# hannes-holey/GaPFlow

Measured on AMD Instinct MI355X. Metric: Mcell-updates/s (fp64), 4096^2 grid, higher is better.
Workload: dtype f64; 1 GPU; 2D journal bearing 4096x4096, fixed DH EOS, all-periodic, adaptive CFL 0.5 (BASELINE.json configs[2]); slabs=1

## Files before the change

gapflow_amd/csrc/api.hip:

```cpp
#include <hip/hip_runtime.h>
#include <algorithm>
#include <cmath>
#include <cstdio>
#include <cstdlib>
#include <cstring>
#include <map>
#include <mutex>
#include <string>
#include <tuple>
#include <vector>

#include "../../include/gapflow_hip.h"
#include "phys_setup.hpp"
#include "step_kernel.hip"
#include "aux_kernels.hip"
#include "step2_kernel.hip"
#include "gp_kernels.hip"
#include "elastic_kernels.hip"
#include "small_kernel.hip"
#include "profile_kernels.hip"

using namespace gpf;

static thread_local std::string g_err;
static const bool g_debug = std::getenv("GPF_DEBUG") != nullptr;
#define DBG(...) do { if (g_debug) { std::fprintf(stderr, "[gpf] " __VA_ARGS__); std::fprintf(stderr, "\n"); std::fflush(stderr); } } while (0)

static int fail(int code, const std::string& msg) {
    g_err = msg;
    return code;
}

struct gpf_handle;
static int enter(gpf_handle* h, bool reads_only = false);

#define HIP_TRY(expr)                                                                                   \
    do {                                                                                                \
        hipError_t e_ = (expr);                                                                         \
        if (e_ != hipSuccess)                                                                           \
            return fail(GPF_ERR_HIP, std::string(#expr) + ": " + hipGetErrorString(e_));               \
    } while (0)

#define GPF_TRY(expr)                                                                                   \
    do {                                                                                                \
        int r_ = (expr);                                                                                \
        if (r_ != GPF_OK) return r_;                                                                    \
    } while (0)

static_assert(sizeof(LogEntry) == sizeof(gpf_scalars_t), "LogEntry must mirror gpf_scalars_t");
static constexpr size_t PLANE_PAD_BYTES = 256;

struct gpf_handle {
    gpf_config cfg;
    Layout L;
    Edges E;
    Phys P;
    hipStream_t stream = nullptr;
    size_t field_bytes = 0;
    double* q[2] = {nullptr, nullptr};
    double* topo = nullptr;
    double* topo_line = nullptr;
    int topo_mode = 0;
    bool topo_hy0 = false;
    double* Ls = nullptr;
    double* g1 = nullptr;
    double* seam = nullptr;
    bool has_seam[2] = {false, false};
    struct { bool on = false; int nranks = 0, rank = 0, rank_lo = -1, rank_hi = -1; char* mine = nullptr;
             char* box[P2P_MAX_RANKS] = {}; unsigned long long* seq = nullptr; } p2p;
    double* halo = nullptr;
    double* beyond = nullptr;
    StepState* st = nullptr;
    Partial* partials = nullptr;
    unsigned int* arrive = nullptr;
    long long p2p_timeout_ticks = P2P_TIMEOUT_TICKS;
    bool split_edges = false;
    bool g1_ready = false;
    Partial* block_partials = nullptr;
    int nghost_blocks = 0;
    ScalarPartial* spart = nullptr;
    int nspart = 0;
    LogEntry* log = nullptr;
    long long log_cap = 0;
    double* stage = nullptr;
    size_t stage_doubles = 0;
    double* fields = nullptr;
    double* work = nullptr;
    struct GpHost {
        bool set = false;
        GpModelDev dev;
        double *Z = nullptr, *alpha = nullptr, *L = nullptr, *Linv = nullptr, *W = nullptr;
        int cap = 0;
        bool has_linv = false;
        double xscale0 = 1.0;
        double inv_scale[GP_MAX_D] = {};
        double yscale_fit = 1.0;
    } gp[3];
    double* gp_state_mean = nullptr;
    bool gp_state_mean_valid = false;
    long long gp_state_mean_step = -1;
    bool gp_state_mean_fresh = false;
    bool open_first_closures = false;
    bool gp_reuse_state_mean = true;
    long long gp_passes[3] = {0, 0, 0}, gp_reused = 0;
    double* gpvar = nullptr;
    double* gpscratch = nullptr;
    int gpscratch_n = 0;
    struct { bool on = false; int px = 0, py = 0, relative = 0; double alpha = 1.0, scale = 1.0; void* plan_f = nullptr; void* plan_b = nullptr;
             double2* greens = nullptr; double2* spec = nullptr; double* dense = nullptr;
             double* u_prev = nullptr; double* h0 = nullptr; double* deformation = nullptr; } el;
    struct { bool on = false; int px = 0, py = 0, nky = 0, nranks = 1, relative = 0;
             int row0 = 0, nrows = 0, k0 = 0, nk = 0, nret = 0, nrows_all = 0, nmain = 0, main_g0 = 0, seam_side = -1, seam_g0 = 0, ref_row = -1;
             double alpha = 1.0, scale = 1.0;
             void* plan_y = nullptr; void* plan_x = nullptr; void* plan_yb = nullptr; int nxg = 0, g_lo = 0;
             double* dense = nullptr; double2* spec = nullptr; double2* send1 = nullptr; double2* recv1 = nullptr; double2* xspec = nullptr;
             double2* greens = nullptr; double2* send2 = nullptr; double2* recv2 = nullptr; double2* line = nullptr; double* ureal = nullptr;
             double* u_prev = nullptr; double* h0 = nullptr; double* deformation = nullptr; double* ref = nullptr; int* rows_all = nullptr; } els;
    double* gptile = nullptr;
    size_t gptile_doubles = 0;
    void* blas = nullptr;
    bool step_open = false;
    int open_parity = 0;
    bool has_q = false, has_topo = false, pre_run_done = false;
    bool prev_state_valid = false;
    long long host_step = 0;
    long long next_step = 0;
    Strip2Geom geom2[2];
    int nchunks2 = 0, nblocks2 = 0, npartials2_cap = 0, nblock_partials_cap = 0;
    bool plan2_valid = false;
    int nt_policy2 = 0;
    int keep_rows2 = 0;
    StepState* st_trial = nullptr;
    double* plan_master = nullptr;
    char plan2_note[400] = "";
};

static int enter(gpf_handle* h, bool reads_only) {
    HIP_TRY(hipSetDevice(h->cfg.device));
    if (!reads_only) h->gp_state_mean_valid = false;
    return GPF_OK;
}

static void make_phys(const gpf_config& c, Phys& P) {
    setup_phys(P, c.U, c.V, c.eta, c.zeta, c.dx, c.dy, c.eos, c.eos_par, c.piezo, c.piezo_par, c.thinning, c.thinning_par);
}

static int blocks_for(long long n, int bs = 256, int cap = 4096) {
    long long b = (n + bs - 1) / bs;
    return (int)std::max<long long>(1, std::min<long long>(b, cap));
}

#ifdef GPF_ONLY_EOS_DH
#define EOS_DISPATCH(eos, ...)                                                                          \
    do {                                                                                                \
        if ((eos) == GPF_EOS_DH) { constexpr int EOS_ = EOS_DH; __VA_ARGS__; }       \
    } while (0)
#else
#define EOS_DISPATCH(eos, ...)                                                                          \
    switch (eos) {                                                                                      \
    case GPF_EOS_DH: { constexpr int EOS_ = EOS_DH; __VA_ARGS__; } break;                              \
    case GPF_EOS_PL: { constexpr int EOS_ = EOS_PL; __VA_ARGS__; } break;                              \
    case GPF_EOS_VDW: { constexpr int EOS_ = EOS_VDW; __VA_ARGS__; } break;                            \
    case GPF_EOS_MT: { constexpr int EOS_ = EOS_MT; __VA_ARGS__; } break;                              \
    case GPF_EOS_CUBIC: { constexpr int EOS_ = EOS_CUBIC; __VA_ARGS__; } break;                        \
    case GPF_EOS_BWR: { constexpr int EOS_ = EOS_BWR; __VA_ARGS__; } break;                            \
    default: { constexpr int EOS_ = EOS_BAYADA; __VA_ARGS__; } break;                                  \
    }
#endif

#define LS_PIEZO_DISPATCH(ls, pz, ...)                                                                  \
    do {                                                                                                \
        if (ls) {                                                                                       \
            constexpr bool LS_ = true;                                                                  \
            if (pz) { constexpr bool PZ_ = true; __VA_ARGS__; } else { constexpr bool PZ_ = false; __VA_ARGS__; }     \
        } else {                                                                                        \
            constexpr bool LS_ = false;                                                                 \
            if (pz) { constexpr bool PZ_ = true; __VA_ARGS__; } else { constexpr bool PZ_ = false; __VA_ARGS__; }     \
        }                                                                                               \
    } while (0)

extern "C" const char* gpf_last_error(void) { return g_err.c_str(); }

extern "C" int gpf_device_count(void) {
    int n = 0;
    if (hipGetDeviceCount(&n) != hipSuccess) return 0;
    return n;
}

static int ensure_stage(gpf_handle* h, size_t doubles) {
    if (h->stage_doubles >= doubles) return GPF_OK;
    if (h->stage) HIP_TRY(hipFree(h->stage));
    h->stage = nullptr; h->stage_doubles = 0;
    HIP_TRY(hipMalloc(&h->stage, doubles * sizeof(double)));
    h->stage_doubles = doubles;
    return GPF_OK;
}

#include "api_fields.inc"

extern "C" int gpf_create(const gpf_config* cfg, gpf_handle** out) {
    if (!cfg || !out) return fail(GPF_ERR_INVALID, "gpf_create: null argument");
    if (cfg->Nx < 1 || cfg->Ny < 1) return fail(GPF_ERR_INVALID, "gpf_create: Nx, Ny must be >= 1");
    if (!(cfg->dx > 0) || !(cfg->dy > 0)) return fail(GPF_ERR_INVALID, "gpf_create: dx, dy must be > 0");
    if (((long long)cfg->Nx + 2) * ((long long)cfg->Ny + 2 + 64) > 2000000000ll)
        return fail(GPF_ERR_INVALID, "gpf_create: more than 2e9 cells per plane; cut the domain into x-slabs (gapflow_amd/slab.py)");
    if (cfg->eos < GPF_EOS_DH || cfg->eos > GPF_EOS_BAYADA) return fail(GPF_ERR_INVALID, "gpf_create: unknown EOS id");
    if (cfg->thinning < 0 || cfg->thinning > GPF_THINNING_CARREAU) return fail(GPF_ERR_INVALID, "gpf_create: unknown shear-thinning id");
    for (int e = 0; e < 4; ++e) {
        int np = 0;
        for (int c = 0; c < 3; ++c) {
            int r = cfg->bc_rule[e][c];
            if (r < 0 || r > 2) return fail(GPF_ERR_INVALID, "gpf_create: bad ghost rule");
            np += (r == GPF_BC_PERIODIC);
        }
        if (np != 0 && np != 3)
            return fail(GPF_ERR_INVALID, "gpf_create: an edge must be periodic for all components or for none "
                                         "(problem.py:682-707 applies the periodic copy only when all three are 'P')");
    }
#ifdef GPF_ONLY_EOS_DH
    if (cfg->eos != GPF_EOS_DH) return fail(GPF_ERR_INVALID, "gpf_create: this build (-DGPF_ONLY_EOS_DH) holds the Dowson-Higginson kernels only");
#endif
    int ndev = 0;
    if (hipGetDeviceCount(&ndev) != hipSuccess || ndev == 0)
        return fail(GPF_ERR_NO_DEVICE, "gpf_create: no HIP device visible (this library has no CPU path)");
    if (cfg->device < 0 || cfg->device >= ndev) return fail(GPF_ERR_INVALID, "gpf_create: device ordinal out of range");
    HIP_TRY(hipSetDevice(cfg->device));

    gpf_handle* h = new gpf_handle();
    h->cfg = *cfg;
    Layout& L = h->L;
    L.Nx = cfg->Nx; L.Ny = cfg->Ny; L.off = 15;
    L.pitch = ((cfg->Ny + 2 + L.off + 15) / 16) * 16;
    if (const char* s = std::getenv("GPF_PITCH_PAD")) L.pitch += (std::atoi(s) / 16) * 16;
    L.plane = (long long)(cfg->Nx + 2) * L.pitch;
    if (const char* s = std::getenv("GPF_PLANE_PAD")) L.plane += (std::atoll(s) & ~1ll);
    for (int e = 0; e < 4; ++e) {
        for (int c = 0; c < 3; ++c) h->E.rule[e][c] = cfg->bc_rule[e][c];
        h->E.value[e] = cfg->bc_value[e];
    }
    h->E.halo[0] = cfg->halo_lo; h->E.halo[1] = cfg->halo_hi;
    h->split_edges = std::getenv("GPF_STEP_UNFUSED_EDGES") != nullptr;
    h->gp_reuse_state_mean = std::getenv("GPF_GP_NO_STATE_MEAN") == nullptr;
    make_phys(*cfg, h->P);

    const size_t plane_b = (size_t)L.plane * sizeof(double);
    auto cleanup = [&](int code) { gpf_destroy(h); return code; };
#define HIP_TRY_C(expr)                                                                                 \
    do {                                                                                                \
        hipError_t e_ = (expr);                                                                         \
        if (e_ != hipSuccess)                                                                           \
            return cleanup(fail(GPF_ERR_HIP, std::string(#expr) + ": " + hipGetErrorString(e_)));      \
    } while (0)
    h->field_bytes = (3 * plane_b + PLANE_PAD_BYTES + 255) & ~(size_t)255;
    for (int b = 0; b < 2; ++b) {
        HIP_TRY_C(field_malloc((void**)&h->q[b], h->field_bytes));
        if (field_zero(0, h->q[b], h->field_bytes) != GPF_OK) { gpf_destroy(h); return GPF_ERR_HIP; }
    }
    HIP_TRY_C(field_malloc((void**)&h->topo, h->field_bytes));
    if (field_zero(0, h->topo, h->field_bytes) != GPF_OK) { gpf_destroy(h); return GPF_ERR_HIP; }
    HIP_TRY_C(hipDeviceSynchronize());
    const size_t g1n = (size_t)3 * L.pitch + (size_t)3 * (L.Nx + 2);
    HIP_TRY_C(hipMalloc(&h->g1, g1n * sizeof(double)));
    HIP_TRY_C(hipMemset(h->g1, 0, g1n * sizeof(double)));
    HIP_TRY_C(hipMalloc(&h->st, sizeof(StepState)));
    HIP_TRY_C(hipMemset(h->st, 0, sizeof(StepState)));
    h->nghost_blocks = std::max(1, std::min(64, (2 * (L.Ny + 2) + 2 * L.Nx + 255) / 256));
    HIP_TRY_C(hipMalloc(&h->arrive, 4 * sizeof(unsigned int)));
    HIP_TRY_C(hipMemset(h->arrive, 0, 4 * sizeof(unsigned int)));
    HIP_TRY_C(hipMalloc(&h->block_partials, 1024 * sizeof(Partial)));
    h->nspart = 1024;
    HIP_TRY_C(hipMalloc(&h->spart, (size_t)(h->nspart + 8) * sizeof(ScalarPartial)));
    HIP_TRY_C(hipMemset(h->spart, 0, (size_t)(h->nspart + 8) * sizeof(ScalarPartial)));
    h->log_cap = 4096;
    HIP_TRY_C(hipMalloc(&h->log, (size_t)h->log_cap * sizeof(LogEntry)));
#undef HIP_TRY_C
    *out = h;
    return GPF_OK;
}

extern "C" int gpf_destroy(gpf_handle* h) {
    if (!h) return GPF_OK;
    hipSetDevice(h->cfg.device);
    hipStreamSynchronize(h->stream);
    for (void* p : {(void*)h->q[0], (void*)h->q[1], (void*)h->topo, (void*)h->plan_master}) field_free(p);
    void* ptrs[] = {h->topo_line, h->Ls, h->g1, h->seam, h->halo, h->beyond, h->st, h->partials, h->arrive, h->block_partials, h->spart,
                    h->log, h->stage, h->fields, h->work, h->st_trial, h->gpvar, h->gp_state_mean, h->gpscratch, h->gptile,
                    h->gp[0].Z, h->gp[0].alpha, h->gp[0].L, h->gp[1].Z, h->gp[1].alpha, h->gp[1].L,
                    h->gp[2].Z, h->gp[2].alpha, h->gp[2].L, h->gp[0].Linv, h->gp[1].Linv, h->gp[2].Linv, h->gp[0].W, h->gp[1].W, h->gp[2].W};
    if (h->blas && roclibs().ok) roclibs().destroy(h->blas);
    if (h->el.plan_f) fftlib().destroy(h->el.plan_f);
    if (h->el.plan_b) fftlib().destroy(h->el.plan_b);
    for (void* p : {(void*)h->el.greens, (void*)h->el.spec, (void*)h->el.dense, (void*)h->el.u_prev})
        if (p) hipFree(p);
    for (void* pl : {h->els.plan_y, h->els.plan_x, h->els.plan_yb})
        if (pl) fftlib().destroy(pl);
    for (void* p : {(void*)h->els.dense, (void*)h->els.spec, (void*)h->els.send1, (void*)h->els.recv1, (void*)h->els.xspec, (void*)h->els.greens,
                    (void*)h->els.send2, (void*)h->els.recv2, (void*)h->els.line, (void*)h->els.ureal, (void*)h->els.u_prev, (void*)h->els.ref,
                    (void*)h->els.rows_all})
        if (p) hipFree(p);
    for (int r = 0; r < h->p2p.nranks; ++r)
        if (h->p2p.box[r] && r != h->p2p.rank) hipIpcCloseMemHandle(h->p2p.box[r]);
    if (h->p2p.mine) hipFree(h->p2p.mine);
    if (h->p2p.seq) hipFree(h->p2p.seq);
    for (void* p : ptrs)
        if (p) hipFree(p);
    delete h;
    return GPF_OK;
}

extern "C" int gpf_set_stream(gpf_handle* h, void* s) {
    if (!h) return fail(GPF_ERR_INVALID, "null handle");
    h->stream = (hipStream_t)s;
    return GPF_OK;
}

static int field_ncomp(int field) {
    switch (field) {
    case GPF_FIELD_Q: return 3;
    case GPF_FIELD_TOPO: return 3;
    case GPF_FIELD_EXTRA: return 1;
    case GPF_FIELD_PRESSURE: return 1;
    case GPF_FIELD_TAU_AVG: return 3;
    case GPF_FIELD_WALL_LOWER: return 6;
    case GPF_FIELD_WALL_UPPER: return 6;
    case GPF_FIELD_PRESSURE_VAR: case GPF_FIELD_WALL_XZ_VAR: case GPF_FIELD_WALL_YZ_VAR: return 1;
    case GPF_FIELD_DEFORMATION: return 1;
    }
    return 0;
}

static int current_parity(gpf_handle* h, int* par) {
    StepState s;
    HIP_TRY(hipMemcpyAsync(&s, h->st, sizeof(s), hipMemcpyDeviceToHost, h->stream));
    HIP_TRY(hipStreamSynchronize(h->stream));
    *par = s.parity;
    return GPF_OK;
}

static int ensure_fields(gpf_handle* h) {
    if (h->fields) return GPF_OK;
    HIP_TRY(hipMalloc(&h->fields, (size_t)16 * h->L.plane * sizeof(double)));
    HIP_TRY(hipMemsetAsync(h->fields, 0, (size_t)16 * h->L.plane * sizeof(double), h->stream));
    return GPF_OK;
}

extern "C" int gpf_upload(gpf_handle* h, int field, const double* host, size_t count) {
    if (!h || !host) return fail(GPF_ERR_INVALID, "gpf_upload: null argument");
    GPF_TRY(enter(h));
    const Layout& L = h->L;
    const int nc = field_ncomp(field);
    if (field != GPF_FIELD_Q && field != GPF_FIELD_TOPO && field != GPF_FIELD_EXTRA)
        return fail(GPF_ERR_INVALID, "gpf_upload: only q, topography and the extra field are inputs");
    const size_t ncell = (size_t)(L.Nx + 2) * (L.Ny + 2);
    if (count != ncell * nc) return fail(GPF_ERR_INVALID, "gpf_upload: count does not match ncomp*(Nx+2)*(Ny+2)");
    double* dst = nullptr;
    if (field == GPF_FIELD_Q) {
        int par = 0;
        GPF_TRY(current_parity(h, &par));
        dst = h->q[par];
    } else if (field == GPF_FIELD_TOPO) {
        dst = h->topo;
    } else {
        bool nz = false;
        for (size_t i = 0; i < count && !nz; ++i) nz = host[i] != 0.0;
        if (!nz && !h->Ls) return GPF_OK;
        if (!h->Ls) { HIP_TRY(hipMalloc(&h->Ls, (size_t)L.plane * sizeof(double) + PLANE_PAD_BYTES)); h->plan2_valid = false; }
        HIP_TRY(hipMemsetAsync(h->Ls, 0, (size_t)L.plane * sizeof(double), h->stream));
        dst = h->Ls;
    }
    if (field == GPF_FIELD_TOPO) {
        const int nx = L.Nx + 2, ny = L.Ny + 2;
        bool xonly = true, yonly = true;
        for (int c = 0; c < 3 && (xonly || yonly); ++c)
            for (int ix = 0; ix < nx && (xonly || yonly); ++ix) {
                const double* row = host + ((size_t)c * nx + ix) * ny;
                const double* row0 = host + (size_t)c * nx * ny;
                for (int iy = 0; iy < ny; ++iy) {
                    if (std::memcmp(&row[iy], &row[0], 8) != 0) xonly = false;
                    if (std::memcmp(&row[iy], &row0[iy], 8) != 0) yonly = false;
                }
            }
        const int mode = xonly ? 1 : (yonly ? 2 : 0);
        if (mode != h->topo_mode) { h->plan2_valid = false; }
        h->topo_mode = (h->el.on || h->els.on) ? 0 : mode;
        if (mode) {
            const int n = mode == 1 ? nx : ny;
            std::vector<double> line((size_t)3 * n);
            for (int c = 0; c < 3; ++c)
                for (int i = 0; i < n; ++i)
                    line[(size_t)c * n + i] = mode == 1 ? host[((size_t)c * nx + i) * ny] : host[(size_t)c * nx * ny + i];
            bool hy0 = mode == 1;
            for (int i = 0; i < n && hy0; ++i) hy0 = line[(size_t)2 * n + i] == 0.0;
            if (hy0 != h->topo_hy0) h->plan2_valid = false;
            h->topo_hy0 = hy0;
            if (!h->topo_line) HIP_TRY(hipMalloc(&h->topo_line, (size_t)3 * (std::max(nx, ny)) * sizeof(double)));
            HIP_TRY(hipMemcpy(h->topo_line, line.data(), line.size() * sizeof(double), hipMemcpyHostToDevice));
        }
    }
    GPF_TRY(ensure_stage(h, count));
    HIP_TRY(hipMemcpyAsync(h->stage, host, count * sizeof(double), hipMemcpyHostToDevice, h->stream));
    hipLaunchKernelGGL(k_pack, dim3(blocks_for((long long)count)), dim3(256), 0, h->stream, h->stage, dst, L, nc);
    HIP_TRY(hipGetLastError());
    HIP_TRY(hipStreamSynchronize(h->stream));
    if (field == GPF_FIELD_Q) h->has_q = true;
    h->g1_ready = false;
    h->prev_state_valid = false;
    if (field == GPF_FIELD_TOPO) h->has_topo = true;
    return GPF_OK;
}

extern "C" int gpf_download(gpf_handle* h, int field, double* host, size_t count) {
    if (!h || !host) return fail(GPF_ERR_INVALID, "gpf_download: null argument");
    GPF_TRY(enter(h, true));
    const Layout& L = h->L;
    const int nc = field_ncomp(field);
    if (nc == 0) return fail(GPF_ERR_INVALID, "gpf_download: unknown field id");
    const size_t ncell = (size_t)(L.Nx + 2) * (L.Ny + 2);
    if (count != ncell * nc) return fail(GPF_ERR_INVALID, "gpf_download: count does not match ncomp*(Nx+2)*(Ny+2)");
    const double* src = nullptr;
    switch (field) {
    case GPF_FIELD_Q: {
        int par = 0;
        GPF_TRY(current_parity(h, &par));
        src = h->q[par];
        break;
    }
    case GPF_FIELD_TOPO: src = h->topo; break;
    case GPF_FIELD_EXTRA:
        if (!h->Ls) { std::memset(host, 0, count * sizeof(double)); return GPF_OK; }
        src = h->Ls; break;
    case GPF_FIELD_DEFORMATION:
        if (!h->el.on && !h->els.on) { std::memset(host, 0, count * sizeof(double)); return GPF_OK; }
        src = h->el.on ? h->el.deformation : h->els.deformation; break;
    case GPF_FIELD_PRESSURE_VAR: case GPF_FIELD_WALL_XZ_VAR: case GPF_FIELD_WALL_YZ_VAR:
        if (!h->gpvar) return fail(GPF_ERR_STATE, "gpf_download: no GP variance has been computed");
        src = h->gpvar + (size_t)(field - GPF_FIELD_PRESSURE_VAR) * L.plane;
        break;
    default:
        if (!h->fields) return fail(GPF_ERR_STATE, "gpf_download: derived fields requested before gpf_update_closures");
        src = h->fields + (field == GPF_FIELD_PRESSURE ? 0 : field == GPF_FIELD_TAU_AVG ? 1 : field == GPF_FIELD_WALL_LOWER ? 4 : 10) * L.plane;
    }
    GPF_TRY(ensure_stage(h, count));
    hipLaunchKernelGGL(k_unpack, dim3(blocks_for((long long)count)), dim3(256), 0, h->stream, src, h->stage, L, nc);
    HIP_TRY(hipGetLastError());
    HIP_TRY(hipMemcpyAsync(host, h->stage, count * sizeof(double), hipMemcpyDeviceToHost, h->stream));
    HIP_TRY(hipStreamSynchronize(h->stream));
    return GPF_OK;
}

static FieldPtrs field_ptrs(gpf_handle* h) {
    FieldPtrs F;
    F.p = h->fields; F.tau = h->fields + h->L.plane; F.lower = h->fields + 4 * h->L.plane; F.upper = h->fields + 10 * h->L.plane;
    return F;
}

static int gp_launch_mean(gpf_handle* h, int which, const double* q, bool with_grad, double* c2_out);
static int read_state(gpf_handle* h, StepState& s);

static const double* beyond_rows(gpf_handle* h, const double* q) {
    if (!h->beyond || (h->E.halo[0] != 1 && h->E.halo[1] != 1)) return nullptr;
    const bool working = h->step_open && q == h->q[h->open_parity ^ 1];
    return h->beyond + (working ? 2 * h->L.pitch : 0);
}

static int launch_fields(gpf_handle* h, const double* q, bool pressure_mean_cached = false) {
    GPF_TRY(ensure_fields(h));
    const Layout& L = h->L;
    const long long n = (long long)(L.Nx + 2) * (L.Ny + 2);
    FieldPtrs F = field_ptrs(h);
    EOS_DISPATCH(h->cfg.eos, {
        if (h->cfg.thinning != GPF_THINNING_NONE) {
            hipLaunchKernelGGL((k_pressure<EOS_>), dim3(blocks_for(n)), dim3(256), 0, h->stream, q, F.p, L, h->P);
            if ((h->E.halo[0] == 1 || h->E.halo[1] == 1) && !h->beyond)
                return fail(GPF_ERR_STATE, "shear thinning on a slab: upload the rows beyond the halo first (gpf_upload_beyond)");
            const double* by = beyond_rows(h, q);
            if (h->Ls) hipLaunchKernelGGL((k_fields_thinning<EOS_, true>), dim3(blocks_for(n)), dim3(256), 0, h->stream, q, h->topo, h->Ls, F, L, h->P, h->cfg.dx, h->cfg.dy, h->E.halo[0], h->E.halo[1], by);
            else hipLaunchKernelGGL((k_fields_thinning<EOS_, false>), dim3(blocks_for(n)), dim3(256), 0, h->stream, q, h->topo, (const double*)nullptr, F, L, h->P, h->cfg.dx, h->cfg.dy, h->E.halo[0], h->E.halo[1], by);
        } else if (h->Ls) hipLaunchKernelGGL((k_fields<EOS_, true>), dim3(blocks_for(n)), dim3(256), 0, h->stream, q, h->topo, h->Ls, F, L, h->P);
        else hipLaunchKernelGGL((k_fields<EOS_, false>), dim3(blocks_for(n)), dim3(256), 0, h->stream, q, h->topo, (const double*)nullptr, F, L, h->P);
    });
    HIP_TRY(hipGetLastError());
    for (int w = 0; w < 3; ++w) {
        if (!h->gp[w].set) continue;
        if (w == 0 && pressure_mean_cached) {
            HIP_TRY(hipMemcpyAsync(F.p, h->gp_state_mean, (size_t)L.plane * sizeof(double), hipMemcpyDeviceToDevice, h->stream));
            h->gp_reused += 1;
        } else GPF_TRY(gp_launch_mean(h, w, q, false, nullptr));
    }
    return GPF_OK;
}

extern "C" int gpf_update_closures(gpf_handle* h) {
    if (!h) return fail(GPF_ERR_INVALID, "null handle");
    if (!h->has_q || !h->has_topo) return fail(GPF_ERR_STATE, "gpf_update_closures: upload q and topography first");
    GPF_TRY(enter(h));
    int par = 0;
    GPF_TRY(current_parity(h, &par));
    if (h->prev_state_valid && !h->E.halo[0] && !h->E.halo[1]) {
        const Layout& L = h->L;
        StepState s;
        GPF_TRY(read_state(h, s));
        double* w = h->q[par ^ 1];
        const long long n = (long long)(L.Nx + 2) * (L.Ny + 2);
        const int nb = blocks_for(n);
        if (!h->work) HIP_TRY(hipMalloc(&h->work, (size_t)9 * L.plane * sizeof(double)));
        GPF_TRY(launch_fields(h, w));
        double *fx = h->work, *fy = h->work + 3 * L.plane, *src = h->work + 6 * L.plane;
        FieldPtrs F = field_ptrs(h);
        const int mc = h->cfg.mc_order;
        const int sw = mc == 0 ? (((s.step - 1) % 2 == 0) ? 1 : -1) : mc;
        const int dir = ((sw + 1) / 2) ? 1 : -1;
        hipLaunchKernelGGL(k_fluxdiff, dim3(nb), dim3(256), 0, h->stream, w, F.p, F.tau, dir, fx, fy, L);
        hipLaunchKernelGGL(k_source, dim3(nb), dim3(256), 0, h->stream, w, h->topo, F.tau, F.lower, F.upper, src, L);
        hipLaunchKernelGGL(k_axpy, dim3(nb), dim3(256), 0, h->stream, w, fx, fy, src, (const double*)&h->st->dt_last, h->cfg.dx, h->cfg.dy, L);
        hipLaunchKernelGGL(k_bc_x, dim3((L.Ny + 2 + 255) / 256), dim3(256), 0, h->stream, w, L, h->E);
        hipLaunchKernelGGL(k_bc_y, dim3((L.Nx + 2 + 255) / 256), dim3(256), 0, h->stream, w, L, h->E);
        HIP_TRY(hipGetLastError());
        GPF_TRY(launch_fields(h, w));
        h->prev_state_valid = false;
    } else {
        GPF_TRY(launch_fields(h, h->q[par]));
    }
    HIP_TRY(hipStreamSynchronize(h->stream));
    return GPF_OK;
}

static int launch_scalars(gpf_handle* h, const double* q, ScalarPartial* total, bool need_sound_speed = true) {
    const Layout& L = h->L;
    const int row0 = h->E.halo[0] == 1 ? 1 : 0, row1 = h->E.halo[1] == 1 ? L.Nx : L.Nx + 1;
    const long long n = (long long)(row1 - row0 + 1) * (L.Ny + 2);
    const int nb = blocks_for(n, 256, h->nspart);
    EOS_DISPATCH(h->cfg.eos, {
        hipLaunchKernelGGL((k_scalars<EOS_>), dim3(nb), dim3(256), 0, h->stream, q, h->topo, L, h->P, row0, row1, h->spart);
    });
    HIP_TRY(hipGetLastError());
    hipLaunchKernelGGL(k_scalars_final, dim3(1), dim3(256), 0, h->stream, h->spart, nb, total);
    HIP_TRY(hipGetLastError());
    if (h->gp[0].set && need_sound_speed) GPF_TRY(gp_launch_mean(h, 0, q, true, &total->c2));
    return GPF_OK;
}

static void fill_scalars(const StepState& s, const ScalarPartial* sp, double dxdy, gpf_scalars_t* out) {
    out->step = s.step; out->simtime = s.simtime; out->dt = s.dt;
    out->ekin = sp ? sp->ekin : s.ekin; out->ekin_old = s.ekin_old; out->residual = s.residual;
    out->v_max = std::sqrt(sp ? sp->v2 : s.vmax2);
    out->v_sound = (sp && ((int)sp->flags & 4)) ? std::nan("") : std::sqrt(sp ? sp->c2 : s.c2max);
    out->mass = sp ? sp->mass * dxdy : 0.0;
    out->invalid = s.invalid; out->converged = s.converged;
}

extern "C" int gpf_scalars(gpf_handle* h, gpf_scalars_t* out) {
    if (!h || !out) return fail(GPF_ERR_INVALID, "gpf_scalars: null argument");
    if (!h->has_q || !h->has_topo) return fail(GPF_ERR_STATE, "gpf_scalars: upload q and topography first");
    GPF_TRY(enter(h, true));
    int par = 0;
    GPF_TRY(current_parity(h, &par));
    ScalarPartial* tot = h->spart + h->nspart;
    h->gp_state_mean_fresh = false;
    GPF_TRY(launch_scalars(h, h->q[par], tot));
    ScalarPartial sp; StepState s;
    HIP_TRY(hipMemcpyAsync(&sp, tot, sizeof(sp), hipMemcpyDeviceToHost, h->stream));
    HIP_TRY(hipMemcpyAsync(&s, h->st, sizeof(s), hipMemcpyDeviceToHost, h->stream));
    HIP_TRY(hipStreamSynchronize(h->stream));
    if (h->gp_state_mean_fresh && s.parity == par) {
        h->gp_state_mean_valid = true;
        h->gp_state_mean_step = s.step;
    }
    h->gp_state_mean_fresh = false;
    fill_scalars(s, &sp, h->cfg.dx * h->cfg.dy, out);
    return GPF_OK;
}

static int write_state(gpf_handle* h, const StepState& s) {
    HIP_TRY(hipMemcpyAsync(h->st, &s, sizeof(s), hipMemcpyHostToDevice, h->stream));
    HIP_TRY(hipStreamSynchronize(h->stream));
    return GPF_OK;
}
static int read_state(gpf_handle* h, StepState& s) {
    HIP_TRY(hipMemcpyAsync(&s, h->st, sizeof(s), hipMemcpyDeviceToHost, h->stream));
    HIP_TRY(hipStreamSynchronize(h->stream));
    return GPF_OK;
}

extern "C" int gpf_set_ekin_old(gpf_handle* h, double v) {
    if (!h) return fail(GPF_ERR_INVALID, "null handle");
    StepState s;
    GPF_TRY(read_state(h, s));
    s.ekin_old = v;
    return write_state(h, s);
}

extern "C" int gpf_set_dt(gpf_handle* h, double dt) {
    if (!h) return fail(GPF_ERR_INVALID, "null handle");
    StepState s;
    GPF_TRY(read_state(h, s));
    s.dt = dt;
    h->g1_ready = false;
    return write_state(h, s);
}

extern "C" int gpf_pre_run(gpf_handle* h) {
    if (!h) return fail(GPF_ERR_INVALID, "null handle");
    if (!h->has_q || !h->has_topo) return fail(GPF_ERR_STATE, "gpf_pre_run: upload q and topography first");
    GPF_TRY(enter(h));
    gpf_scalars_t sc;
    GPF_TRY(gpf_scalars(h, &sc));
    StepState s;
    GPF_TRY(read_state(h, s));
    const gpf_config& c = h->cfg;
    s.hmin = std::min(c.dx, c.dy);
    s.tol = c.tol; s.CFL = c.CFL; s.adaptive = c.adaptive; s.mc_order = c.mc_order; s.max_it = c.max_it;
    s.step = 0; s.simtime = 0.0; s.residual = 1.0;
    s.rbuf[0] = 1.0; s.rcount = 1; s.rhead = 0;
    s.converged = (1.0 < c.tol) ? 1 : 0;
    s.invalid = 0;
    s.dt_last = 0.0;
    if (!h->pre_run_done) s.ekin_old = sc.ekin;
    s.ekin = sc.ekin;
    s.vmax2 = sc.v_max * sc.v_max; s.c2max = sc.v_sound * sc.v_sound;
    const double dt_crit = s.hmin / (sc.v_max + sc.v_sound);
    s.dt = c.adaptive ? c.CFL * dt_crit : c.dt_fixed;
    GPF_TRY(write_state(h, s));
    h->pre_run_done = true;
    h->g1_ready = false;
    h->prev_state_valid = false;
    h->host_step = 0; h->next_step = 0;
    return GPF_OK;
}

static int topo_mode_of(const gpf_handle* h) {
    if (h->Ls != nullptr || h->cfg.piezo != 0 || std::getenv("GPF_TOPO_PLANES")) return 0;
    if (h->topo_mode == 1 && h->topo_hy0 && !std::getenv("GPF_TOPO_GENERIC")) return 3;
    return h->topo_mode;
}

typedef void (*step2_kernel_t)(const Step2Args, const Phys);

static step2_kernel_t step2_kernel(int eos, bool has_ls, bool piezo, int D, int topo_mode) {
    step2_kernel_t k = nullptr;
    EOS_DISPATCH(eos, {
        if (piezo) {
            if (has_ls) k = D > 0 ? k_step2<EOS_, true, true, 1, 0> : k_step2<EOS_, true, true, -1, 0>;
            else k = D > 0 ? k_step2<EOS_, false, true, 1, 0> : k_step2<EOS_, false, true, -1, 0>;
        } else if (has_ls) {
            k = D > 0 ? k_step2<EOS_, true, false, 1, 0> : k_step2<EOS_, true, false, -1, 0>;
        } else if (topo_mode == 1) {
            k = D > 0 ? k_step2<EOS_, false, false, 1, 1> : k_step2<EOS_, false, false, -1, 1>;
        } else if (topo_mode == 2) {
            k = D > 0 ? k_step2<EOS_, false, false, 1, 2> : k_step2<EOS_, false, false, -1, 2>;
        } else if (topo_mode == 3) {
            k = D > 0 ? k_step2<EOS_, false, false, 1, 3> : k_step2<EOS_, false, false, -1, 3>;
        } else {
            k = D > 0 ? k_step2<EOS_, false, false, 1, 0> : k_step2<EOS_, false, false, -1, 0>;
        }
    });
    return k;
}

static Strip2Geom strip2_geom(const Layout& L, int D) {
    Strip2Geom G;
    const int e = (D < 0 && (L.Ny & 1)) ? 1 : 0;
    for (int k = 0; k < 2; ++k) {
        G.w0 = -1 - e - 4 * k;
        G.s_ghost = (L.Ny - G.w0 - 1) / STRIP2;
        const int p_ny = L.Ny - G.w0 - STRIP2 * G.s_ghost;
        G.lane_ghost = (p_ny + 1) >> 1; G.slot_ghost = (p_ny + 1) & 1;
        if (G.lane_ghost + 2 <= 63) break;
    }
    G.nstrips = G.s_ghost + 1;
    G.lane_wrap = G.lane_ghost + 1;
    const int p0 = -G.w0;
    G.wrap_ma = (p0 % 2 == 0) ? 0 : -1;
    const int d = 1 - G.wrap_ma;
    G.wrap_src_lane = G.lane_wrap + d / 2; G.wrap_src_slot = d & 1;
    return G;
}

static bool step2_fused(const gpf_handle* h) { return !h->split_edges; }

#include "api_plan.inc"

#ifndef GPF_SLAB_COMMIT_BLOCKS
#define GPF_SLAB_COMMIT_BLOCKS 24
#endif
constexpr int SLAB_COMMIT_BLOCKS = GPF_SLAB_COMMIT_BLOCKS;

static P2PArgs p2p_args(gpf_handle* h, bool on) {
    P2PArgs c;
    c.on = on ? 1 : 0; c.nranks = h->p2p.nranks; c.rank = h->p2p.rank; c.rank_lo = h->p2p.rank_lo; c.rank_hi = h->p2p.rank_hi;
    for (int r = 0; r < P2P_MAX_RANKS; ++r) c.box[r] = h->p2p.box[r];
    c.seq = h->p2p.seq; c.qa = h->q[0]; c.qb = h->q[1];
    return c;
}

static int ghost_args(gpf_handle* h, int honor_stop, GhostArgs& g) {
    const Layout& L = h->L;
    g.qa = h->q[0]; g.qb = h->q[1]; g.topo = h->topo; g.Ls = h->Ls;
    for (int e = 0; e < 2; ++e) {
        g.seam[e] = nullptr;
        if (h->E.halo[e] == 2) {
            if (!h->has_seam[e]) return fail(GPF_ERR_STATE, "periodic slab seam: call gpf_set_seam_topo for this edge first");
            g.seam[e] = h->seam + (size_t)e * 8 * L.pitch;
        }
    }
    g.g1x = h->g1; g.g1y = h->g1 + 3 * L.pitch;
    g.st = h->st; g.L = L; g.E = h->E; g.honor_stop = honor_stop;
    return GPF_OK;
}

static void fill_step2_args(gpf_handle* h, Step2Args& a2, int D, int honor_stop, long long log_base, double* slab_out, bool p2p) {
    const Layout& L = h->L;
    const bool fused = step2_fused(h);
    const Strip2Geom& G2 = h->geom2[D > 0 ? 0 : 1];
    a2.qa = h->q[0]; a2.qb = h->q[1]; a2.topo = h->topo; a2.topo_line = h->topo_line; a2.Ls = h->Ls;
    a2.g1x = h->g1; a2.g1y = h->g1 + 3 * L.pitch;
    a2.st = h->st; a2.partials = h->partials; a2.block_partials = h->block_partials; a2.arrive = h->arrive;
    a2.log = h->log; a2.log_base = log_base; a2.log_cap = h->log_cap;
    a2.L = L; a2.E = h->E; a2.G = G2; a2.nchunks = h->nchunks2; a2.fused = (fused ? 1 : 0) | (h->nt_policy2 >= 1 ? 2 : 0) | (h->nt_policy2 >= 2 ? 4 : 0) |
               (h->nt_policy2 >= 1 ? h->keep_rows2 << 3 : 0); a2.honor_stop = honor_stop;
    const bool slab = slab_out != nullptr;
    for (int e = 0; e < 2; ++e) a2.seam[e] = (h->E.halo[e] == 2 && h->has_seam[e]) ? h->seam + (size_t)e * 8 * L.pitch : nullptr;
    a2.out = slab_out; a2.msg = (slab && !p2p) ? h->halo : nullptr; a2.p2p = p2p_args(h, p2p);
}

static int enqueue_step(gpf_handle* h, int honor_stop, long long log_base, double* slab_out,
                        hipEvent_t ev0 = nullptr, hipEvent_t ev1 = nullptr, bool p2p = false) {
    const Layout& L = h->L;
    const int mc = h->cfg.mc_order;
    const int D = mc == 0 ? ((h->next_step % 2 == 0) ? 1 : -1) : (((mc + 1) / 2) ? 1 : -1);
    GPF_TRY(plan_step2(h, D));
    h->next_step += 1;
    const bool fused = step2_fused(h);
    const Strip2Geom& G2 = h->geom2[D > 0 ? 0 : 1];
    const int np_step = G2.nstrips * h->nchunks2;
    GhostArgs g;
    GPF_TRY(ghost_args(h, honor_stop, g));
    Step2Args a2;
    fill_step2_args(h, a2, D, honor_stop, log_base, slab_out, p2p);
    const bool slab = slab_out != nullptr;
    FinishArgs f;
    f.partials = h->partials; f.st = h->st;
    f.log = h->log; f.log_base = log_base; f.log_cap = h->log_cap; f.out = slab_out; f.honor_stop = honor_stop;
    f.L = L; f.E = h->E;
    f.p2p = p2p_args(h, p2p);
    f.arrive = h->arrive; f.msg = slab ? h->halo : nullptr;
    f.nstep_partials = np_step; f.block_partials = h->block_partials;
    GhostFillArgs gf;
    gf.qa = h->q[0]; gf.qb = h->q[1]; gf.st = h->st;
    gf.L = L; gf.E = h->E; gf.honor_stop = honor_stop;

    const int ntiles = (L.Nx + L.Ny + 63) / 64;
    const dim3 ggrid(std::min(ntiles, 512));
    const int nsend = slab ? std::min((6 * L.pitch + 1023) / 1024, 256) : 0;
    WaitArgs w;
    w.qa = h->q[0]; w.qb = h->q[1]; w.st = h->st; w.log = h->log; w.log_base = log_base; w.log_cap = h->log_cap;
    w.L = L; w.E = h->E; w.honor_stop = honor_stop; w.arrive = h->arrive + 1; w.timeout_ticks = h->p2p_timeout_ticks; w.p2p = f.p2p;
    w.gathered = nullptr; w.msg_len = 0; w.nranks = 0; w.rank_lo = w.rank_hi = -1; w.stage1 = fused ? 0 : 1;
    const bool has_ls = h->Ls != nullptr;
    if (fused) {
        const step2_kernel_t k2 = step2_kernel(h->cfg.eos, h->Ls != nullptr, h->cfg.piezo != 0, D, topo_mode_of(h));
        if (ev0) hipEventRecord(ev0, h->stream);
        hipLaunchKernelGGL(k2, dim3(h->nblocks2), dim3(256), 0, h->stream, a2, h->P);
        if (ev1) hipEventRecord(ev1, h->stream);
        if (p2p) {
            const dim3 cgrid(SLAB_COMMIT_BLOCKS);
            EOS_DISPATCH(h->cfg.eos, {
                hipLaunchKernelGGL((k_begin_slab<EOS_, false, false, false, true>), cgrid, dim3(256), 0, h->stream, g, w, h->P);
            });
        }
        h->g1_ready = false;
        HIP_TRY(hipGetLastError());
        return GPF_OK;
    }
    EOS_DISPATCH(h->cfg.eos, {
        if (!h->g1_ready) {
            if (topo_mode_of(h) == 3) hipLaunchKernelGGL((k_ghost_stage1<EOS_, false, false, true>), ggrid, dim3(256), 0, h->stream, g, h->P);
            else LS_PIEZO_DISPATCH(has_ls, h->cfg.piezo != 0, hipLaunchKernelGGL((k_ghost_stage1<EOS_, LS_, PZ_, false>), ggrid, dim3(256), 0, h->stream, g, h->P));
        }
        if (ev0) hipEventRecord(ev0, h->stream);
        hipLaunchKernelGGL(step2_kernel(h->cfg.eos, h->Ls != nullptr, h->cfg.piezo != 0, D, topo_mode_of(h)), dim3(h->nblocks2), dim3(256), 0, h->stream, a2, h->P);
        if (ev1) hipEventRecord(ev1, h->stream);
        hipLaunchKernelGGL((k_ghost_fill<EOS_>), dim3(h->nghost_blocks + nsend), dim3(256), 0, h->stream, gf, f, h->nghost_blocks, h->P);
        if (p2p) {
            if (topo_mode_of(h) == 3) hipLaunchKernelGGL((k_begin_slab<EOS_, false, false, true, true>), ggrid, dim3(256), 0, h->stream, g, w, h->P);
            else LS_PIEZO_DISPATCH(has_ls, h->cfg.piezo != 0, hipLaunchKernelGGL((k_begin_slab<EOS_, LS_, PZ_, false, true>), ggrid, dim3(256), 0, h->stream, g, w, h->P));
        }
    });
    h->g1_ready = p2p;
    HIP_TRY(hipGetLastError());
    return GPF_OK;
}

static bool small_grid_eligible(gpf_handle* h) {
    static const bool off = getenv("GPF_SMALL_GRID") && atoi(getenv("GPF_SMALL_GRID")) == 0;
    const long long nc = (long long)(h->L.Nx + 2) * (h->L.Ny + 2);
    return !off && nc * SMALL_DOUBLES_PER_CELL * 8 <= 150 * 1024 && h->cfg.thinning == GPF_THINNING_NONE && !h->E.halo[0] && !h->E.halo[1] &&
           !h->gp[0].set && !h->gp[1].set && !h->gp[2].set && !h->el.on;
}

static int enqueue_small_steps(gpf_handle* h, int nsteps, int honor_stop, long long log_base) {
    const Layout& L = h->L;
    SmallArgs a;
    a.qa = h->q[0]; a.qb = h->q[1]; a.topo = h->topo; a.Ls = h->Ls; a.st = h->st;
    a.log = h->log; a.log_base = log_base; a.log_cap = h->log_cap; a.L = L; a.E = h->E; a.nsteps = nsteps; a.honor_stop = honor_stop;
    const size_t lds = (size_t)(L.Nx + 2) * (L.Ny + 2) * SMALL_DOUBLES_PER_CELL * 8;
    EOS_DISPATCH(h->cfg.eos, {
        if (h->Ls) {
            HIP_TRY(hipFuncSetAttribute((const void*)k_small_steps<EOS_, true>, hipFuncAttributeMaxDynamicSharedMemorySize, (int)lds));
            hipLaunchKernelGGL((k_small_steps<EOS_, true>), dim3(1), dim3(512), lds, h->stream, a, h->P);
        } else {
            HIP_TRY(hipFuncSetAttribute((const void*)k_small_steps<EOS_, false>, hipFuncAttributeMaxDynamicSharedMemorySize, (int)lds));
            hipLaunchKernelGGL((k_small_steps<EOS_, false>), dim3(1), dim3(512), lds, h->stream, a, h->P);
        }
    });
    HIP_TRY(hipGetLastError());
    h->next_step += nsteps;
    h->g1_ready = false;
    return GPF_OK;
}

extern "C" int gpf_step(gpf_handle* h, int64_t n, int honor_stop, gpf_scalars_t* log, int64_t log_capacity,
                        int64_t* n_executed) {
    if (!h) return fail(GPF_ERR_INVALID, "null handle");
    if (!h->pre_run_done) return fail(GPF_ERR_STATE, "gpf_step: call gpf_pre_run first (Problem._pre_run, problem.py:412)");
    if (h->E.halo[0] || h->E.halo[1]) return fail(GPF_ERR_STATE, "gpf_step: this handle is a slab; use gpf_step_local / gpf_step_commit");
    if (h->cfg.thinning != GPF_THINNING_NONE)
        return fail(GPF_ERR_STATE, "gpf_step: shear thinning needs grad p (a wider stencil than the fused step has); use the stage-wise calls");
    if (n < 0) return fail(GPF_ERR_INVALID, "gpf_step: n < 0");
    GPF_TRY(enter(h));
    int64_t done = 0, logged = 0;
    const bool small = small_grid_eligible(h);
    while (done < n) {
        const int64_t batch = std::min<int64_t>(n - done, h->log_cap);
        const long long base = h->host_step;
        if (small) GPF_TRY(enqueue_small_steps(h, (int)batch, honor_stop, base));
        else for (int64_t i = 0; i < batch; ++i) GPF_TRY(enqueue_step(h, honor_stop, base, nullptr));
        StepState s;
        GPF_TRY(read_state(h, s));
        const long long ran = s.step - base;
        const long long entries = ran + ((s.invalid && ran < batch) ? 1 : 0);
        if (log && entries > 0) {
            const long long take = std::min<long long>(entries, log_capacity - logged);
            if (take > 0) {
                HIP_TRY(hipMemcpy(log + logged, h->log, (size_t)take * sizeof(LogEntry), hipMemcpyDeviceToHost));
                logged += take;
            }
        }
        h->host_step = s.step; h->next_step = s.step;
        h->prev_state_valid = ran >= 1 && !s.invalid;
        done += batch;
        if (ran < batch) break;
    }
    if (n_executed) *n_executed = h->host_step;
    return GPF_OK;
}

extern "C" int gpf_step_timed(gpf_handle* h, int64_t n, double* kernel_ms, double* total_ms) {
    if (!h || !kernel_ms || !total_ms) return fail(GPF_ERR_INVALID, "gpf_step_timed: null argument");
    if (!h->pre_run_done) return fail(GPF_ERR_STATE, "gpf_step_timed: call gpf_pre_run first");
    if (n < 1 || n > h->log_cap) return fail(GPF_ERR_INVALID, "gpf_step_timed: 1 <= n <= 4096");
    GPF_TRY(enter(h));
    std::vector<hipEvent_t> ev(2 * n + 2);
    for (auto& e : ev) HIP_TRY(hipEventCreate(&e));
    HIP_TRY(hipEventRecord(ev[2 * n], h->stream));
    int rc = GPF_OK;
    for (int64_t i = 0; i < n && rc == GPF_OK; ++i) rc = enqueue_step(h, 0, h->host_step, nullptr, ev[2 * i], ev[2 * i + 1]);
    HIP_TRY(hipEventRecord(ev[2 * n + 1], h->stream));
    HIP_TRY(hipStreamSynchronize(h->stream));
    double sum = 0.0;
    float ms = 0.f;
    for (int64_t i = 0; i < n; ++i) {
        HIP_TRY(hipEventElapsedTime(&ms, ev[2 * i], ev[2 * i + 1]));
        sum += ms;
    }
    HIP_TRY(hipEventElapsedTime(&ms, ev[2 * n], ev[2 * n + 1]));
    *kernel_ms = sum; *total_ms = ms;
    for (auto& e : ev) hipEventDestroy(e);
    StepState s;
    GPF_TRY(read_state(h, s));
    h->prev_state_valid = s.step > h->host_step && !s.invalid;
    h->host_step = s.step; h->next_step = s.step;
    return rc;
}

#include "api_unfused_step.inc"
#include "api_operators.inc"
#include "api_slab_allgather.inc"
#include "api_elastic.inc"
#include "api_slab_p2p.inc"
#include "api_gp.inc"
#include "api_stagewise.inc"
#include "api_slab_stagewise.inc"
#include "api_slab_elastic.inc"
#include "api_profiles.inc"
```

gapflow_amd/csrc/api_plan.inc:

```

constexpr int K2_LONG_MARCH_ROWS = 100;

static int plan_apply(gpf_handle* h, int nchunks, int nt, int keep = 0) {
    const Layout& L = h->L;
    const int nstrips = std::max(h->geom2[0].nstrips, h->geom2[1].nstrips);
    nchunks = std::max(1, std::min(nchunks, std::max(1, L.Nx / 4)));
    h->nchunks2 = nchunks;
    h->nt_policy2 = nt;
    h->keep_rows2 = nt >= 1 ? std::max(0, std::min(7, keep)) : 0;
    const int nwaves = nstrips * nchunks;
    h->nblocks2 = (((nwaves + 3) / 4) + 7) / 8 * 8;
    if (nwaves > h->npartials2_cap) {
        if (h->partials) HIP_TRY(hipFree(h->partials));
        h->partials = nullptr;
        HIP_TRY(hipMalloc(&h->partials, (size_t)nwaves * sizeof(Partial)));
        HIP_TRY(hipMemset(h->partials, 0, (size_t)nwaves * sizeof(Partial)));
        h->npartials2_cap = nwaves;
    }
    if (h->nblocks2 > h->nblock_partials_cap) {
        const int cap = std::max(1024, h->nblocks2);
        if (h->block_partials) HIP_TRY(hipFree(h->block_partials));
        h->block_partials = nullptr;
        HIP_TRY(hipMalloc(&h->block_partials, (size_t)cap * sizeof(Partial)));
        h->nblock_partials_cap = cap;
    }
    return GPF_OK;
}

static void fill_step2_args(gpf_handle* h, Step2Args& a2, int D, int honor_stop, long long log_base, double* slab_out, bool p2p);

static int plan_trial(gpf_handle* h, int D, float* us, int reps = 6, bool both = false) {
    static const int parity_value[2] = {0, 1};
    if (!h->st_trial) HIP_TRY(hipMalloc(&h->st_trial, sizeof(StepState)));
    h->prev_state_valid = false;
    both = both && h->plan_master != nullptr;
    int par = 0;
    if (both) GPF_TRY(current_parity(h, &par));
    Step2Args a2;
    fill_step2_args(h, a2, D, 0, 0, nullptr, false);
    a2.st = h->st_trial; a2.log = nullptr;
    const step2_kernel_t k2 = step2_kernel(h->cfg.eos, h->Ls != nullptr, h->cfg.piezo != 0, D, topo_mode_of(h));
    hipEvent_t e0, e1;
    HIP_TRY(hipEventCreate(&e0)); HIP_TRY(hipEventCreate(&e1));
    float total = 0.f;
    for (int r = -1; r < reps; ++r) {
        HIP_TRY(hipMemcpyAsync(h->st_trial, h->st, sizeof(StepState), hipMemcpyDeviceToDevice, h->stream));
        if (both && ((r + 1) & 1))
            HIP_TRY(hipMemcpyAsync(&h->st_trial->parity, &parity_value[par ^ 1], sizeof(int), hipMemcpyHostToDevice, h->stream));
        HIP_TRY(hipEventRecord(e0, h->stream));
        hipLaunchKernelGGL(k2, dim3(h->nblocks2), dim3(256), 0, h->stream, a2, h->P);
        HIP_TRY(hipEventRecord(e1, h->stream));
        HIP_TRY(hipEventSynchronize(e1));
        float ms = 0.f;
        HIP_TRY(hipEventElapsedTime(&ms, e0, e1));
        if (r >= 0) total += ms;
    }
    hipEventDestroy(e0); hipEventDestroy(e1);
    if (both) GPF_TRY(field_copy(h->stream, h->q[par], h->plan_master, h->field_bytes));
    HIP_TRY(hipGetLastError());
    *us = total / reps * 1e3f;
    return GPF_OK;
}

static float placement_best_seen(const gpf_handle* h, int D, float mine) {
    static std::mutex lock;
    static std::map<std::tuple<int, int, int, int, int, int, int>, float> seen;
    const auto key = std::make_tuple(h->L.Nx, h->L.Ny, h->cfg.eos, topo_mode_of(h), D, h->Ls ? 1 : 0, h->cfg.piezo != 0 ? 1 : 0);
    std::lock_guard<std::mutex> g(lock);
    float& v = seen[key];
    if (mine > 0.f && (v == 0.f || mine < v)) v = mine;
    return v;
}

static int plan_placement(gpf_handle* h, int D, std::string& note) {
    const char* env_tries = std::getenv("GPF_PLACEMENT_TRIES");
    const int fixed = env_tries ? std::atoi(env_tries) : -1;
    if (fixed == 0 || !h->plan_master) return GPF_OK;
    const bool print = std::getenv("GPF_PLACEMENT_PRINT") && std::atoi(std::getenv("GPF_PLACEMENT_PRINT")) != 0;
    int par = 0;
    GPF_TRY(current_parity(h, &par));
    const bool planes = topo_mode_of(h) == 0;
    double* const master = h->plan_master;
    std::vector<double*> pool = {h->q[par], h->q[par ^ 1]};
    std::vector<char> holds_state = {1, 0};
    std::vector<float> w = {0.f, 0.f};
    auto trial = [&](int i, int j, float* us, bool both) -> int {
        if (!holds_state[i]) {
            GPF_TRY(field_copy(h->stream, pool[i], master, h->field_bytes));
            holds_state[i] = 1;
        }
        holds_state[j] = 0;
        h->q[par] = pool[i]; h->q[par ^ 1] = pool[j];
        return plan_trial(h, D, us, 6, both);
    };
    float best_w = 0.f;
    for (int round = 0; round < (fixed > 0 ? 1 : 5); ++round) {
        int want = fixed > 0 ? fixed : 12;
        size_t free_b = 0, total_b = 0;
        HIP_TRY(hipMemGetInfo(&free_b, &total_b));
        while (want > 0 && (size_t)want * h->field_bytes + (2ull << 30) > free_b) --want;
        const size_t first = pool.size();
        for (int k = 0; k < want; ++k) {
            double* b = nullptr;
            if (field_malloc((void**)&b, h->field_bytes) != hipSuccess) { (void)hipGetLastError(); break; }
            GPF_TRY(field_zero(h->stream, b, h->field_bytes));
            pool.push_back(b); holds_state.push_back(0); w.push_back(0.f);
        }
        if (pool.size() == first) break;
        float batch_best = 0.f;
        for (size_t k = first; k < pool.size(); ++k) {
            GPF_TRY(trial(0, (int)k, &w[k], false));
            if (batch_best == 0.f || w[k] < batch_best) batch_best = w[k];
        }
        const bool paid = best_w == 0.f || batch_best < 0.99f * best_w;
        if (best_w == 0.f || batch_best < best_w) best_w = batch_best;
        const float known = placement_best_seen(h, D, 0.f);
        if (round >= 1 && !paid && !(known > 0.f && best_w > 1.03f * known)) break;
    }
    (void)placement_best_seen(h, D, best_w);
    const int n = (int)pool.size();
    if (n == 2) return GPF_OK;
    GPF_TRY(trial(0, 1, &w[1], false));
    GPF_TRY(trial(1, 0, &w[0], false));
    std::vector<int> order(n);
    for (int k = 0; k < n; ++k) order[k] = k;
    std::stable_sort(order.begin(), order.end(), [&](int x, int y) { return w[x] < w[y]; });
    const int m = std::min(n, 4);
    float own_pair = 0.f;
    GPF_TRY(trial(0, 1, &own_pair, true));
    int bi = 0, bj = 1;
    float best = own_pair, worst = own_pair;
    std::string pairs;
    for (int i = 0; i < m; ++i)
        for (int j = i + 1; j < m; ++j) {
            const int x = std::min(order[i], order[j]), y = std::max(order[i], order[j]);
            if (x == 0 && y == 1) continue;
            float t = 0.f;
            GPF_TRY(trial(x, y, &t, true));
            if (print) { char b2[40]; std::snprintf(b2, sizeof b2, " (%d,%d) %.1f", x, y, t); pairs += b2; }
            if (t < best) { best = t; bi = x; bj = y; }
            worst = std::max(worst, t);
        }
    if (print) {
        std::fprintf(stderr, "[gpf] placement: us per step writing each buffer (0, 1: the handle's own):");
        for (int k = 0; k < n; ++k) std::fprintf(stderr, " %.1f", w[k]);
        std::fprintf(stderr, "\n[gpf] placement: pairs, both directions: (0,1) %.1f%s\n", own_pair, pairs.c_str());
    }
    char buf[200];
    std::snprintf(buf, sizeof buf, " placement: %d buffers, written %.0f .. %.0f us, pair kept %.0f, the handle's own %.0f", n,
                  *std::min_element(w.begin(), w.end()), *std::max_element(w.begin(), w.end()), best, own_pair);
    note = buf;
    std::vector<double*> rest;
    for (int k = 0; k < n; ++k) if (k != bi && k != bj) rest.push_back(pool[k]);
    float us = 0.f;
    if (planes) {
        double* const own = h->topo;
        double* best_home = own;
        float best_t = 0.f;
        std::string seen;
        for (size_t k = 0; k <= std::min<size_t>(rest.size(), 3); ++k) {
            double* cand = k == 0 ? own : rest[k - 1];
            if (cand != own) GPF_TRY(field_copy(h->stream, cand, own, h->field_bytes));
            h->topo = cand;
            float t = 0.f;
            GPF_TRY(trial(bi, bj, &t, true));
            std::snprintf(buf, sizeof buf, " %.0f", t);
            seen += buf;
            if (k == 0 || t < best_t) { best_t = t; best_home = cand; }
        }
        note += "; gap planes:" + seen;
        if (best_home != own) {
            rest.erase(std::find(rest.begin(), rest.end(), best_home));
            rest.push_back(own);
        }
        h->topo = best_home;
    }
    GPF_TRY(trial(bi, bj, &us, true));
    HIP_TRY(hipStreamSynchronize(h->stream));
    for (double* b : rest) field_free(b);
    h->q[par] = pool[bi]; h->q[par ^ 1] = pool[bj];
    return GPF_OK;
}

static const char* const NT_NAME[3] = {"plain loads and stores", "non-temporal stores", "non-temporal loads and stores"};
constexpr int K2_KEEP_ROWS_DEFAULT = 4;
static const int K2_KEEP_CANDIDATES[2] = {3, 4};
static std::string keep_note(const gpf_handle* h) {
    if (h->nt_policy2 < 1) return "";
    char buf[64];
    std::snprintf(buf, sizeof buf, ", keep %d/8 rows on-die", h->keep_rows2);
    return buf;
}
static int plan_step2(gpf_handle* h, int D) {
    if (h->plan2_valid) return GPF_OK;
    const Layout& L = h->L;
    h->geom2[0] = strip2_geom(L, 1);
    h->geom2[1] = strip2_geom(L, -1);
    const int nstrips = std::max(h->geom2[0].nstrips, h->geom2[1].nstrips);
    int per_cu = 0, ncu = 0;
    HIP_TRY(hipOccupancyMaxActiveBlocksPerMultiprocessor(&per_cu, (const void*)step2_kernel(h->cfg.eos, h->Ls != nullptr, h->cfg.piezo != 0, 1, topo_mode_of(h)), 256, 0));
    HIP_TRY(hipDeviceGetAttribute(&ncu, hipDeviceAttributeMultiprocessorCount, h->cfg.device));
    const int all_resident = std::max(1, std::max(1, per_cu * ncu) * 4 / nstrips);
    const int one_per_simd = (ncu * 4) / nstrips;
    const double streamed = (double)L.plane * 8.0 * (6 + (topo_mode_of(h) == 0 ? 3 : 0) + (h->Ls ? 1 : 0));
    const bool nt_possible = streamed > 192.0 * 1024 * 1024;
    const char* env_chunks = std::getenv("GPF_CHUNKS");
    const char* env_nt = std::getenv("GPF_NT") ? std::getenv("GPF_NT") : std::getenv("GPF_NT_STORES");
    const char* env_tune = std::getenv("GPF_PLAN_TUNE");
    int nchunks = all_resident;
    if (one_per_simd >= 1 && L.Nx / one_per_simd >= K2_LONG_MARCH_ROWS) nchunks = one_per_simd;
    int nt = nt_possible ? 2 : 0;
    if (env_chunks && std::atoi(env_chunks) > 0) nchunks = std::atoi(env_chunks);
    if (env_nt) nt = std::max(0, std::min(2, std::atoi(env_nt)));
    const char* env_keep = std::getenv("GPF_KEEP_ROWS");
    int keep = nt_possible ? K2_KEEP_ROWS_DEFAULT : 0;
    if (env_keep) keep = std::max(0, std::min(7, std::atoi(env_keep)));
    const bool tune = !(env_tune && std::atoi(env_tune) == 0) && !h->split_edges && h->pre_run_done && (long long)L.Nx * L.Ny >= (1ll << 20) &&
                      one_per_simd >= 1 && L.Nx / one_per_simd >= 16 && !(env_chunks && env_nt);
    if (!tune) {
        GPF_TRY(plan_apply(h, nchunks, nt, keep));
        std::snprintf(h->plan2_note, sizeof h->plan2_note, "%d chunks per strip, %s%s (rule of thumb%s)", h->nchunks2,
                      NT_NAME[h->nt_policy2], keep_note(h).c_str(), (env_chunks || env_nt || env_keep) ? ", pinned by the environment" : "");
        h->plan2_valid = true;
        return GPF_OK;
    }
    std::string placement_note;
    GPF_TRY(plan_apply(h, nchunks, nt));
    {
        int par = 0;
        GPF_TRY(current_parity(h, &par));
        if (field_malloc((void**)&h->plan_master, h->field_bytes) == hipSuccess)
            GPF_TRY(field_copy(h->stream, h->plan_master, h->q[par], h->field_bytes));
        else { (void)hipGetLastError(); h->plan_master = nullptr; }
    }
    {
        float unused = 0.f;
        const double step_s = 1.1e-11 * (double)L.Nx * L.Ny + 1e-5;
        GPF_TRY(plan_trial(h, D, &unused, (int)std::min(200.0, std::max(8.0, 0.012 / step_s))));
    }
    float best = 0.f;
    int best_chunks = nchunks;
    int best_nt = nt;
    int best_keep = 0;
    std::string seen, keep_seen;
    auto pick_plan = [&]() -> int {
        best = 0.f;
        seen.clear();
        for (int c : {one_per_simd, all_resident}) {
            if (env_chunks && std::atoi(env_chunks) > 0) c = std::atoi(env_chunks);
            for (int pol = 0; pol < (nt_possible && !env_nt ? 3 : 1); ++pol) {
                const int cand_nt = env_nt ? nt : pol;
                GPF_TRY(plan_apply(h, c, cand_nt));
                float us = 0.f;
                GPF_TRY(plan_trial(h, D, &us, 6, true));
                char buf[48];
                std::snprintf(buf, sizeof buf, " %d/%s %.0f", h->nchunks2, cand_nt == 2 ? "nt" : cand_nt == 1 ? "nts" : "plain", us);
                seen += buf;
                if (best == 0.f || us < best) { best = us; best_chunks = c; best_nt = cand_nt; }
            }
            if ((env_chunks && std::atoi(env_chunks) > 0) || one_per_simd == all_resident) break;
        }
        best_keep = 0;
        keep_seen.clear();
        if (best_nt >= 1) {
            if (env_keep) best_keep = keep;
            else if (nt_possible) {
                char buf[48];
                std::snprintf(buf, sizeof buf, " 0 %.0f", best);
                keep_seen = buf;
                float best_k = best;
                for (int k : K2_KEEP_CANDIDATES) {
                    GPF_TRY(plan_apply(h, best_chunks, best_nt, k));
                    float us = 0.f;
                    GPF_TRY(plan_trial(h, D, &us, 6, true));
                    std::snprintf(buf, sizeof buf, ", %d %.0f", k, us);
                    keep_seen += buf;
                    if (us < best_k) { best_k = us; best_keep = k; }
                }
            }
        }
        return plan_apply(h, best_chunks, best_nt, best_keep);
    };
    const bool verify = std::getenv("GPF_PLACEMENT_PRINT") && std::atoi(std::getenv("GPF_PLACEMENT_PRINT")) >= 2;
    auto stamp = [&](const char* when) {
        if (!verify) return;
        int par = 0;
        if (current_parity(h, &par) != GPF_OK) return;
        std::fprintf(stderr, "[gpf] %-28s q[par] %p %016llx   master %p %016llx\n", when, (void*)h->q[par], field_checksum(h->stream, h->q[par], h->field_bytes),
                     (void*)h->plan_master, h->plan_master ? field_checksum(h->stream, h->plan_master, h->field_bytes) : 0ull);
    };
    stamp("before the first plan");
    GPF_TRY(pick_plan());
    stamp("after the first plan");
    const std::string first_seen = seen;
    GPF_TRY(plan_placement(h, D, placement_note));
    stamp("after the placement");
    if (!placement_note.empty()) GPF_TRY(pick_plan());
    stamp("after the second plan");
    HIP_TRY(hipStreamSynchronize(h->stream));
    field_free(h->plan_master);
    h->plan_master = nullptr;
    GPF_TRY(plan_apply(h, best_chunks, best_nt, best_keep));
    const std::string kept = keep_note(h) + (keep_seen.empty() ? (env_keep && h->nt_policy2 >= 1 ? " (pinned by the environment)" : "")
                                                               : " (timed, us: k" + keep_seen + ")");
    std::snprintf(h->plan2_note, sizeof h->plan2_note, "%d chunks per strip, %s%s (timed, us:%s;%s%s%s)", h->nchunks2,
                  NT_NAME[h->nt_policy2], kept.c_str(), seen.c_str(), placement_note.c_str(),
                  placement_note.empty() ? "" : "; before the placement:", placement_note.empty() ? "" : first_seen.c_str());
    DBG("plan_step2: %s", h->plan2_note);
    h->plan2_valid = true;
    return GPF_OK;
}

extern "C" const char* gpf_plan_note(gpf_handle* h) { return h ? h->plan2_note : ""; }
```

gapflow_amd/csrc/aux_kernels.hip:

```cpp
#include <hip/hip_runtime.h>
#include "device_types.hpp"

namespace gpf {

__global__ void k_pack(const double* __restrict__ src, double* __restrict__ dst, Layout L, int ncomp) {
    const long long ncell = (long long)(L.Nx + 2) * (L.Ny + 2);
    for (long long i = blockIdx.x * (long long)blockDim.x + threadIdx.x; i < ncell * ncomp;
         i += (long long)gridDim.x * blockDim.x) {
        const int c = (int)(i / ncell);
        const long long r = i - c * ncell;
        const int ix = (int)(r / (L.Ny + 2)), iy = (int)(r - (long long)ix * (L.Ny + 2));
        dst[c * L.plane + L.at(ix, iy)] = src[i];
    }
}

__global__ void k_unpack(const double* __restrict__ src, double* __restrict__ dst, Layout L, int ncomp) {
    const long long ncell = (long long)(L.Nx + 2) * (L.Ny + 2);
    for (long long i = blockIdx.x * (long long)blockDim.x + threadIdx.x; i < ncell * ncomp;
         i += (long long)gridDim.x * blockDim.x) {
        const int c = (int)(i / ncell);
        const long long r = i - c * ncell;
        const int ix = (int)(r / (L.Ny + 2)), iy = (int)(r - (long long)ix * (L.Ny + 2));
        dst[i] = src[c * L.plane + L.at(ix, iy)];
    }
}

__device__ __forceinline__ double ghost_x(const double* q, const Layout& L, const Edges& E, int e, int c, int iy) {
    const int r = E.rule[e][c];
    const int adj = e == 0 ? 1 : L.Nx;
    const int src = (r == BC_P) ? (e == 0 ? L.Nx : 1) : adj;
    const double v = q[c * L.plane + L.at(src, iy)];
    return r == BC_D ? 2.0 * E.value[e] - v : v;
}
__device__ __forceinline__ double ghost_y(const double* q, const Layout& L, const Edges& E, int e, int c, int ix) {
    const int r = E.rule[e][c];
    const int adj = e == 2 ? 1 : L.Ny;
    const int src = (r == BC_P) ? (e == 2 ? L.Ny : 1) : adj;
    const double v = q[c * L.plane + L.at(ix, src)];
    return r == BC_D ? 2.0 * E.value[e] - v : v;
}

__global__ void k_bc_x(double* q, Layout L, Edges E) {
    const int iy = blockIdx.x * blockDim.x + threadIdx.x;
    if (iy > L.Ny + 1) return;
    for (int e = 0; e < 2; ++e) {
        if (E.halo[e]) continue;
        const int ix = e == 0 ? 0 : L.Nx + 1;
        double v[3];
        for (int c = 0; c < 3; ++c) v[c] = ghost_x(q, L, E, e, c, iy);
        for (int c = 0; c < 3; ++c) q[c * L.plane + L.at(ix, iy)] = v[c];
    }
}
__global__ void k_bc_y(double* q, Layout L, Edges E) {
    const int ix = blockIdx.x * blockDim.x + threadIdx.x;
    if (ix > L.Nx + 1) return;
    for (int e = 2; e < 4; ++e) {
        const int iy = e == 2 ? 0 : L.Ny + 1;
        double v[3];
        for (int c = 0; c < 3; ++c) v[c] = ghost_y(q, L, E, e, c, ix);
        for (int c = 0; c < 3; ++c) q[c * L.plane + L.at(ix, iy)] = v[c];
    }
}

struct Acc {
    double ekin, v2, c2, mass;
    int flags;
    __device__ __forceinline__ void zero() { ekin = 0; v2 = 0; c2 = 0; mass = 0; flags = 0; }
    template <int EOS>
    __device__ __forceinline__ void cell(double r, double jx, double jy, double h, const Phys& P, double w = 1.0) {
        const double v = (jx * jx + jy * jy) / r;
        ekin += w * (v * 0.5);
        v2 = nanmax(v2, v);
        const double c = eos_c2<EOS>(r, P);
        if (!(c >= 0.0)) flags |= 4;
        c2 = fmax(c2, c);
        mass += w * (r * h);
        if (r != r || jx != jx || jy != jy) flags |= 1;
        if (r < 0.0) flags |= 2;
    }
    __device__ __forceinline__ void merge(const Acc& o) {
        ekin += o.ekin; v2 = nanmax(v2, o.v2); c2 = nanmax(c2, o.c2); mass += o.mass; flags |= o.flags;
    }
};

__device__ __forceinline__ Acc wave_reduce(Acc a) {
    for (int s = 32; s >= 1; s >>= 1) {
        Acc o;
        o.ekin = __shfl_down(a.ekin, s); o.v2 = __shfl_down(a.v2, s); o.c2 = __shfl_down(a.c2, s);
        o.mass = __shfl_down(a.mass, s); o.flags = __shfl_down(a.flags, s);
        a.merge(o);
    }
    return a;
}

__device__ __forceinline__ Acc block_reduce(Acc a, Acc* smem) {
    a = wave_reduce(a);
    const int lane = threadIdx.x & 63, w = threadIdx.x >> 6;
    if (lane == 0) smem[w] = a;
    __syncthreads();
    Acc r; r.zero();
    if (threadIdx.x == 0) {
        for (int i = 0; i < (int)(blockDim.x >> 6); ++i) r.merge(smem[i]);
    }
    __syncthreads();
    return r;
}

struct ScalarPartial { double ekin, v2, c2, mass, flags; };

template <int EOS>
__global__ __launch_bounds__(256) void k_scalars(const double* q, const double* topo, Layout L, Phys P, int row0,
                                                 int row1, ScalarPartial* out) {
    __shared__ Acc sm[4];
    Acc a; a.zero();
    const long long w = L.Ny + 2;
    const long long n = (long long)(row1 - row0 + 1) * w;
    for (long long i = blockIdx.x * (long long)blockDim.x + threadIdx.x; i < n; i += (long long)gridDim.x * blockDim.x) {
        const int ix = row0 + (int)(i / w), iy = (int)(i % w);
        const long long o = L.at(ix, iy);
        a.cell<EOS>(q[o], q[o + L.plane], q[o + 2 * L.plane], topo[o], P);
    }
    a = block_reduce(a, sm);
    if (threadIdx.x == 0) {
        ScalarPartial p = {a.ekin, a.v2, a.c2, a.mass, (double)a.flags};
        out[blockIdx.x] = p;
    }
}

__device__ __forceinline__ double critical_dt(const StepState* st, double v2, double c2) {
    return st->hmin / (sqrt(v2) + sqrt(c2));
}

__device__ inline void commit_step(StepState* st, double ekin, double v2, double c2, int flags, LogEntry* log,
                                   long long log_base, long long log_cap) {
    if (flags & 4) c2 = __builtin_nan("");
    flags &= 3;
    if (flags) {
        st->invalid = (flags & 1) ? 1 : 2;
    } else {
        const double dt_crit = critical_dt(st, v2, c2);
        const double cfl = st->dt / dt_crit;
        const double res = fabs(ekin - st->ekin_old) / st->ekin_old / cfl;
        st->residual = res;
        if (st->rcount < 5) { st->rbuf[st->rcount++] = res; }
        else { st->rbuf[st->rhead] = res; st->rhead = (st->rhead + 1) % 5; }
        bool conv = true;
        for (int i = 0; i < st->rcount; ++i) conv = conv && (st->rbuf[i] < st->tol);
        st->converged = conv ? 1 : 0;
        st->ekin_old = ekin;
        st->ekin = ekin; st->vmax2 = v2; st->c2max = c2;
        st->step += 1;
        st->simtime += st->dt;
        st->dt_last = st->dt;
        if (st->adaptive) st->dt = st->CFL * dt_crit;
        st->parity ^= 1;
    }
    if (log) {
        const long long k = (flags ? st->step : st->step - 1) - log_base;
        if (k >= 0 && k < log_cap) {
            LogEntry e;
            e.step = st->step; e.simtime = st->simtime; e.dt = st->dt; e.ekin = st->ekin; e.ekin_old = st->ekin_old;
            e.residual = st->residual; e.v_max = sqrt(st->vmax2); e.v_sound = sqrt(st->c2max); e.mass = 0.0;
            e.invalid = st->invalid; e.converged = st->converged;
            log[k] = e;
        }
    }
}

constexpr long long P2P_TIMEOUT_TICKS = 3000000000ll;
constexpr int P2P_MAX_RANKS = 16;
constexpr size_t P2P_ROWS_OFFSET = 4096;
struct MailHeader {
    unsigned long long flag[2][P2P_MAX_RANKS];
    double rec[2][P2P_MAX_RANKS][8];
};
__host__ __device__ inline size_t p2p_mailbox_bytes(int pitch) { return P2P_ROWS_OFFSET + (size_t)2 * 2 * 3 * pitch * sizeof(double); }
__device__ inline double* p2p_rows(char* box, int slot, int side, int pitch) {
    return (double*)(box + P2P_ROWS_OFFSET) + (size_t)(slot * 2 + side) * 3 * pitch;
}
struct P2PArgs {
    int on, nranks, rank, rank_lo, rank_hi;
    char* box[P2P_MAX_RANKS];
    unsigned long long* seq;
    const double* qa; const double* qb;
};

struct FinishArgs {
    const Partial* partials;
    StepState* st;
    LogEntry* log; long long log_base, log_cap;
    double* out;
    int honor_stop;
    Layout L; Edges E;
    int nstep_partials;
    Partial* block_partials;
    unsigned int* arrive;
    double* msg;
    P2PArgs p2p;
};

#ifdef GPF_STRICT_ATOMICS
#define GPF_ORDER_ARRIVE __ATOMIC_ACQ_REL
#define GPF_ORDER_LOAD __ATOMIC_ACQUIRE
#else
#define GPF_ORDER_ARRIVE __ATOMIC_RELAXED
#define GPF_ORDER_LOAD __ATOMIC_RELAXED
#endif

__device__ __forceinline__ void publish_partial(Partial* slot, const Acc& acc) {
    unsigned long long* w = reinterpret_cast<unsigned long long*>(slot);
    __hip_atomic_store(w + 0, (unsigned long long)__double_as_longlong(acc.ekin), __ATOMIC_RELAXED, __HIP_MEMORY_SCOPE_AGENT);
    __hip_atomic_store(w + 1, (unsigned long long)__double_as_longlong(acc.v2), __ATOMIC_RELAXED, __HIP_MEMORY_SCOPE_AGENT);
    __hip_atomic_store(w + 2, (unsigned long long)__double_as_longlong(acc.c2), __ATOMIC_RELAXED, __HIP_MEMORY_SCOPE_AGENT);
    __hip_atomic_store(w + 3, (unsigned long long)__double_as_longlong((double)acc.flags), __ATOMIC_RELAXED, __HIP_MEMORY_SCOPE_AGENT);
    asm volatile("s_waitcnt vmcnt(0)" ::: "memory");
}
__device__ __forceinline__ void merge_published(Acc& acc, const Partial* slot) {
    const unsigned long long* w = reinterpret_cast<const unsigned long long*>(slot);
    const double ekin = __longlong_as_double((long long)__hip_atomic_load(w + 0, GPF_ORDER_LOAD, __HIP_MEMORY_SCOPE_AGENT));
    const double v2 = __longlong_as_double((long long)__hip_atomic_load(w + 1, GPF_ORDER_LOAD, __HIP_MEMORY_SCOPE_AGENT));
    const double c2 = __longlong_as_double((long long)__hip_atomic_load(w + 2, GPF_ORDER_LOAD, __HIP_MEMORY_SCOPE_AGENT));
    const double fl = __longlong_as_double((long long)__hip_atomic_load(w + 3, GPF_ORDER_LOAD, __HIP_MEMORY_SCOPE_AGENT));
    acc.ekin += ekin; acc.v2 = nanmax(acc.v2, v2); acc.c2 = nanmax(acc.c2, c2); acc.flags |= (int)fl;
}

__device__ inline void finish_tail(StepState* st, LogEntry* log, long long log_base, long long log_cap, double* out,
                                   const Partial* block_partials, const P2PArgs& p2p, Acc* sm) {
    __shared__ double rec_sm[8];
    Acc acc; acc.zero();
    for (int i = threadIdx.x; i < (int)gridDim.x; i += blockDim.x) merge_published(acc, block_partials + i);
    acc = block_reduce(acc, sm);
    if (threadIdx.x == 0) {
        if (out) {
            const double inf = __builtin_inf();
            out[0] = acc.ekin;
            out[1] = acc.v2 != acc.v2 ? inf : acc.v2;
            out[2] = acc.c2 != acc.c2 ? inf : acc.c2;
            out[3] = (double)acc.flags;
            out[4] = out[5] = out[6] = out[7] = 0.0;
            for (int k = 0; k < 8; ++k) rec_sm[k] = out[k];
        } else {
            commit_step(st, acc.ekin, acc.v2, acc.c2, acc.flags, log, log_base, log_cap);
        }
    }
    if (p2p.on) {
        __syncthreads();
        const P2PArgs& c = p2p;
        const unsigned long long n = *c.seq + 1;
        const int slot = (int)(n & 1);
        if (threadIdx.x < c.nranks) {
            MailHeader* hd = (MailHeader*)c.box[threadIdx.x];
            for (int k = 0; k < 8; ++k) hd->rec[slot][c.rank][k] = rec_sm[k];
            __hip_atomic_store(&hd->flag[slot][c.rank], n, __ATOMIC_RELEASE, __HIP_MEMORY_SCOPE_SYSTEM);
        }
    }
}

__device__ inline void finish_tail(const FinishArgs& a, Acc* sm) {
    finish_tail(a.st, a.log, a.log_base, a.log_cap, a.out, a.block_partials, a.p2p, sm);
}

__device__ inline void finish_step(const FinishArgs& f, Acc own, Acc* sm) {
    __shared__ int last;
    const int per = (f.nstep_partials + (int)gridDim.x - 1) / (int)gridDim.x;
    const int i0 = blockIdx.x * per, i1 = min(i0 + per, f.nstep_partials);
    for (int i = i0 + threadIdx.x; i < i1; i += blockDim.x) {
        const Partial p = f.partials[i];
        own.ekin += p.ekin; own.v2 = nanmax(own.v2, p.vmax2); own.c2 = nanmax(own.c2, p.c2max); own.flags |= (int)p.flags;
    }
    own = block_reduce(own, sm);
    if (threadIdx.x == 0) {
        publish_partial(f.block_partials + blockIdx.x, own);
        last = __hip_atomic_fetch_add(f.arrive, 1u, GPF_ORDER_ARRIVE, __HIP_MEMORY_SCOPE_AGENT) == gridDim.x - 1 ? 1 : 0;
        if (last) __hip_atomic_store(f.arrive, 0u, __ATOMIC_RELAXED, __HIP_MEMORY_SCOPE_AGENT);
    }
    __syncthreads();
    if (!last) return;
    finish_tail(f, sm);
}

__device__ inline void send_rows_block(const double* q, const FinishArgs& f, int sblock, int nsblocks) {
    const Layout& L = f.L;
    double *dst_first, *dst_last;
    if (f.p2p.on) {
        const P2PArgs& c = f.p2p;
        const int slot = (int)((*c.seq + 1) & 1);
        dst_first = (c.rank_lo >= 0 && f.E.halo[0]) ? p2p_rows(c.box[c.rank_lo], slot, 1, L.pitch) : nullptr;
        dst_last = (c.rank_hi >= 0 && f.E.halo[1]) ? p2p_rows(c.box[c.rank_hi], slot, 0, L.pitch) : nullptr;
    } else {
        dst_first = f.msg; dst_last = f.msg + 3 * L.pitch;
    }
    const int total = 6 * L.pitch;
    for (int t = sblock * blockDim.x + threadIdx.x; t < total; t += nsblocks * blockDim.x) {
        const int side = t / (3 * L.pitch), k = (t / L.pitch) % 3, i = t % L.pitch;
        double* dst = side ? dst_last : dst_first;
        if (!dst) continue;
        const int ix = side ? L.Nx : 1, iy = i - L.off;
        double v = 0.0;
        if (iy >= 1 && iy <= L.Ny) v = q[k * L.plane + (long long)ix * L.pitch + i];
        else if (iy == 0 || iy == L.Ny + 1) v = ghost_y(q, L, f.E, iy == 0 ? 2 : 3, k, ix);
        if (f.p2p.on)
            __hip_atomic_store(reinterpret_cast<unsigned long long*>(dst + k * L.pitch + i), (unsigned long long)__double_as_longlong(v),
                               __ATOMIC_RELAXED, __HIP_MEMORY_SCOPE_SYSTEM);
        else dst[k * L.pitch + i] = v;
    }
    if (f.p2p.on) asm volatile("s_waitcnt vmcnt(0)" ::: "memory");
}

struct GhostFillArgs {
    double* qa; double* qb;
    const StepState* st;
    Layout L; Edges E;
    int honor_stop;
};

template <int EOS>
__device__ __forceinline__ Acc ghost_fill_block(const GhostFillArgs& a, const Phys& P, int block, int nblocks) {
    const Layout& L = a.L;
    double* q = a.st->parity ? a.qa : a.qb;
    Acc acc; acc.zero();
    auto put = [&](int ix, int iy, const double v[3], double w) {
        const long long o = L.at(ix, iy);
        q[o] = v[0]; q[o + L.plane] = v[1]; q[o + 2 * L.plane] = v[2];
        acc.cell<EOS>(v[0], v[1], v[2], 0.0, P, w);
    };
    const int nrow = 2 * (L.Ny + 2), ncol = 2 * L.Nx;
    for (int t = block * blockDim.x + threadIdx.x; t < nrow + ncol; t += nblocks * blockDim.x) {
        double v[3];
        if (t < nrow) {
            const int e = t / (L.Ny + 2), iy = t % (L.Ny + 2);
            if (a.E.halo[e]) continue;
            const int ix = e == 0 ? 0 : L.Nx + 1;
            if (iy >= 1 && iy <= L.Ny) {
                for (int c = 0; c < 3; ++c) v[c] = ghost_x(q, L, a.E, e, c, iy);
            } else {
                const int ey = iy == 0 ? 2 : 3;
                const int r0 = a.E.rule[ey][0];
                const int src = (r0 == BC_P) ? (ey == 2 ? L.Ny : 1) : (ey == 2 ? 1 : L.Ny);
                for (int c = 0; c < 3; ++c) {
                    const double gx = ghost_x(q, L, a.E, e, c, src);
                    v[c] = a.E.rule[ey][c] == BC_D ? 2.0 * a.E.value[ey] - gx : gx;
                }
            }
            put(ix, iy, v, 1.0);
        } else {
            const int u = t - nrow;
            const int e = 2 + u / L.Nx, ix = 1 + u % L.Nx;
            for (int c = 0; c < 3; ++c) v[c] = ghost_y(q, L, a.E, e, c, ix);
            const double w = 1.0 + ((ix == 1 && a.E.halo[0] == 2) ? 1.0 : 0.0) + ((ix == L.Nx && a.E.halo[1] == 2) ? 1.0 : 0.0);
            put(ix, e == 2 ? 0 : L.Ny + 1, v, w);
        }
    }
    return acc;
}

template <int EOS>
__global__ __launch_bounds__(256) void k_ghost_fill(const GhostFillArgs a, const FinishArgs f, int nfill, const Phys P) {
    __shared__ Acc sm[4];
    const StepState* st = a.st;
    if (st->invalid != 0 || (a.honor_stop && (st->converged || st->step >= st->max_it))) return;
    Acc own; own.zero();
    if ((int)blockIdx.x < nfill) own = ghost_fill_block<EOS>(a, P, blockIdx.x, nfill);
    else send_rows_block(st->parity ? a.qa : a.qb, f, blockIdx.x - nfill, gridDim.x - nfill);
    finish_step(f, own, sm);
}


struct HaloArgs {
    double* qa; double* qb;
    double* msg;
    const double* gathered;
    int rank_lo, rank_hi;
    const StepState* st;
    Layout L; Edges E;
    int honor_stop;
    int work_parity;
    double* beyond;
    int msg_rows;
};
__global__ void k_halo_pack(const HaloArgs a) {
    if (a.st->invalid != 0 || (a.honor_stop && (a.st->converged || a.st->step >= a.st->max_it))) return;
    const double* q = a.work_parity >= 0 ? (a.work_parity ? a.qb : a.qa) : (a.st->parity ? a.qa : a.qb);
    const int i = blockIdx.x * blockDim.x + threadIdx.x;
    if (i >= a.L.pitch) return;
    for (int c = 0; c < 3; ++c) {
        a.msg[c * a.L.pitch + i] = q[c * a.L.plane + (long long)1 * a.L.pitch + i];
        a.msg[(3 + c) * a.L.pitch + i] = q[c * a.L.plane + (long long)a.L.Nx * a.L.pitch + i];
    }
    if (a.msg_rows == 8) {
        a.msg[6 * a.L.pitch + i] = q[(long long)min(2, a.L.Nx) * a.L.pitch + i];
        a.msg[7 * a.L.pitch + i] = q[(long long)max(a.L.Nx - 1, 1) * a.L.pitch + i];
    }
}
__global__ void k_halo_unpack(const HaloArgs a) {
    if (a.st->invalid != 0 || (a.honor_stop && (a.st->converged || a.st->step >= a.st->max_it))) return;
    double* q = a.work_parity >= 0 ? (a.work_parity ? a.qb : a.qa) : (a.st->parity ? a.qa : a.qb);
    const int i = blockIdx.x * blockDim.x + threadIdx.x;
    if (i >= a.L.pitch) return;
    const long long len = (long long)a.msg_rows * a.L.pitch + 8;
    for (int c = 0; c < 3; ++c) {
        if (a.E.halo[0] && a.rank_lo >= 0) q[c * a.L.plane + i] = a.gathered[a.rank_lo * len + (3 + c) * a.L.pitch + i];
        if (a.E.halo[1] && a.rank_hi >= 0)
            q[c * a.L.plane + (long long)(a.L.Nx + 1) * a.L.pitch + i] = a.gathered[a.rank_hi * len + c * a.L.pitch + i];
    }
    if (a.beyond) {
        if (a.E.halo[0] && a.rank_lo >= 0) a.beyond[i] = a.gathered[a.rank_lo * len + 7 * a.L.pitch + i];
        if (a.E.halo[1] && a.rank_hi >= 0) a.beyond[a.L.pitch + i] = a.gathered[a.rank_hi * len + 6 * a.L.pitch + i];
    }
}

__global__ void k_beyond_average(double* state, const double* work, int n) {
    const int i = blockIdx.x * blockDim.x + threadIdx.x;
    if (i < n) state[i] = (work[i] + state[i]) / 2.0;
}

constexpr int INVALID_PEER_TIMEOUT = 3;
struct WaitArgs {
    double* qa; double* qb;
    StepState* st;
    LogEntry* log; long long log_base, log_cap;
    Layout L; Edges E;
    int honor_stop;
    unsigned int* arrive;
    long long timeout_ticks;
    P2PArgs p2p;
    const double* gathered;
    long long msg_len;
    int nranks, rank_lo, rank_hi;
    int stage1;
};
template <int EOS, bool HAS_LS, bool PIEZO, bool XONLY, bool MAILBOX>
__global__ __launch_bounds__(256) void k_begin_slab(const GhostArgs g, const WaitArgs a, const Phys P) {
    __shared__ int missing, last;
    __shared__ double tiles[2][3][64];
    StepState* st = a.st;
    if (st->invalid != 0 || (a.honor_stop && (st->converged || st->step >= st->max_it))) return;
    const P2PArgs& c = a.p2p;
    const unsigned long long n = MAILBOX ? *c.seq + 1 : 0ull;
    const int slot = (int)(n & 1);
    MailHeader* hd = MAILBOX ? (MailHeader*)c.box[c.rank] : nullptr;
    const int nranks = MAILBOX ? c.nranks : a.nranks, rank_lo = MAILBOX ? c.rank_lo : a.rank_lo, rank_hi = MAILBOX ? c.rank_hi : a.rank_hi;
    if (threadIdx.x == 0) missing = 0;
    __syncthreads();
    if (MAILBOX && threadIdx.x < c.nranks) {
        const long long t0 = wall_clock64();
        bool ok = false;
        int probes = 0;
        for (;;) {
            ok = __hip_atomic_load(&hd->flag[slot][threadIdx.x], __ATOMIC_RELAXED, __HIP_MEMORY_SCOPE_SYSTEM) >= n;
            if (ok) break;
            __builtin_amdgcn_s_sleep(2);
            if ((++probes & 255) == 0 && wall_clock64() - t0 > a.timeout_ticks) break;
        }
        if (!ok) atomicAdd(&missing, 1);
        __builtin_amdgcn_fence(__ATOMIC_ACQUIRE, "");
    }
    __syncthreads();
    const bool timed_out = missing != 0;
    double ekin = 0.0, v2 = 0.0, c2 = 0.0;
    int flags = 0;
    const Layout& L = a.L;
    for (int r = 0; r < nranks; ++r) {
        const double* p = MAILBOX ? hd->rec[slot][r] : a.gathered + r * a.msg_len + 6ll * L.pitch;
        ekin += p[0];
        v2 = fmax(v2, p[1]); c2 = fmax(c2, p[2]);
        flags |= (int)p[3];
    }
    const double inf = __builtin_inf();
    if (v2 == inf) v2 = __builtin_nan("");
    if (c2 == inf) c2 = __builtin_nan("");
    const int nblocks = gridDim.x * gridDim.y, block = blockIdx.y * gridDim.x + blockIdx.x;
    if (!timed_out && (flags & 3) == 0) {
        double* q = st->parity ? a.qa : a.qb;
        const double* row_lo = !(rank_lo >= 0 && a.E.halo[0]) ? nullptr
                             : MAILBOX ? p2p_rows(c.box[c.rank], slot, 0, L.pitch) : a.gathered + rank_lo * a.msg_len + 3ll * L.pitch;
        const double* row_hi = !(rank_hi >= 0 && a.E.halo[1]) ? nullptr
                             : MAILBOX ? p2p_rows(c.box[c.rank], slot, 1, L.pitch) : a.gathered + rank_hi * a.msg_len;
        for (int t = block * blockDim.x + threadIdx.x; t < 6 * L.pitch; t += nblocks * blockDim.x) {
            const int side = t / (3 * L.pitch), k = (t / L.pitch) % 3, i = t % L.pitch;
            const double* src = side ? row_hi : row_lo;
            if (src) q[k * L.plane + (long long)(side ? L.Nx + 1 : 0) * L.pitch + i] = src[k * L.pitch + i];
        }
        if (a.stage1) {
        const double c2_eff = (flags & 4) ? __builtin_nan("") : c2;
        const double dt = st->adaptive ? st->CFL * critical_dt(st, v2, c2_eff) : st->dt;
        const int D = direction_of_step(st, st->step + 1);
        MailField fld;
        fld.q = q; fld.L = L; fld.row_lo = row_lo; fld.row_hi = row_hi;
        const int ntiles = (L.Ny + L.Nx + 63) / 64;
        for (int tile = block; tile < ntiles; tile += nblocks) ghost_stage1_tile<EOS, HAS_LS, PIEZO, XONLY>(fld, g, P, D, tile * 64, dt, tiles);
        }
    }
    __syncthreads();
    if (threadIdx.x == 0) {
        if (timed_out) {
            __hip_atomic_fetch_add(a.arrive + 1, 1u, __ATOMIC_RELAXED, __HIP_MEMORY_SCOPE_AGENT);
            asm volatile("s_waitcnt vmcnt(0)" ::: "memory");
        }
        last = __hip_atomic_fetch_add(a.arrive, 1u, GPF_ORDER_ARRIVE, __HIP_MEMORY_SCOPE_AGENT) == (unsigned)nblocks - 1 ? 1 : 0;
    }
    __syncthreads();
    if (last && threadIdx.x == 0) {
        const unsigned int misses = __hip_atomic_load(a.arrive + 1, __ATOMIC_RELAXED, __HIP_MEMORY_SCOPE_AGENT);
        __hip_atomic_store(a.arrive, 0u, __ATOMIC_RELAXED, __HIP_MEMORY_SCOPE_AGENT);
        __hip_atomic_store(a.arrive + 1, 0u, __ATOMIC_RELAXED, __HIP_MEMORY_SCOPE_AGENT);
        if (misses) {
            st->invalid = INVALID_PEER_TIMEOUT;
        } else {
            if (MAILBOX) *c.seq = n;
            commit_step(st, ekin, v2, c2, flags, a.log, a.log_base, a.log_cap);
        }
    }
}

__global__ void k_record_unfused(const ScalarPartial* pre, const ScalarPartial* post, double* rec) {
    const double inf = __builtin_inf();
    rec[0] = post->ekin;
    rec[1] = post->v2 != post->v2 ? inf : post->v2;
    rec[2] = post->c2 != post->c2 ? inf : post->c2;
    rec[3] = (double)(((int)pre->flags & 3) | ((int)post->flags & 4));
    rec[4] = rec[5] = rec[6] = rec[7] = 0.0;
}

__global__ void k_commit_gathered(StepState* st, const double* gathered, long long len, long long rec_off, int nranks,
                                  LogEntry* log, long long log_base, long long log_cap, int honor_stop) {
    if (st->invalid != 0 || (honor_stop && (st->converged || st->step >= st->max_it))) return;
    double ekin = 0.0, v2 = 0.0, c2 = 0.0;
    int flags = 0;
    for (int r = 0; r < nranks; ++r) {
        const double* p = gathered + r * len + rec_off;
        ekin += p[0];
        v2 = fmax(v2, p[1]); c2 = fmax(c2, p[2]);
        flags |= (int)p[3];
    }
    const double inf = __builtin_inf();
    if (v2 == inf) v2 = __builtin_nan("");
    if (c2 == inf) c2 = __builtin_nan("");
    commit_step(st, ekin, v2, c2, flags, log, log_base, log_cap);
}

__global__ __launch_bounds__(256) void k_scalars_final(const ScalarPartial* in, int n, ScalarPartial* out) {
    __shared__ Acc sm[4];
    Acc a; a.zero();
    for (int i = threadIdx.x; i < n; i += blockDim.x) {
        Acc o; o.ekin = in[i].ekin; o.v2 = in[i].v2; o.c2 = in[i].c2; o.mass = in[i].mass; o.flags = (int)in[i].flags;
        a.merge(o);
    }
    a = block_reduce(a, sm);
    if (threadIdx.x == 0) {
        ScalarPartial p = {a.ekin, a.v2, a.c2, a.mass, (double)a.flags};
        out[0] = p;
    }
}

struct FieldPtrs {
    double* p;
    double* tau;
    double* lower;
    double* upper;
};

template <int EOS, bool HAS_LS>
__global__ __launch_bounds__(256) void k_fields(const double* q, const double* topo, const double* Ls, FieldPtrs F,
                                                Layout L, Phys P) {
    const long long w = L.Ny + 2, n = (long long)(L.Nx + 2) * w;
    for (long long i = blockIdx.x * (long long)blockDim.x + threadIdx.x; i < n; i += (long long)gridDim.x * blockDim.x) {
        const long long o = L.at((int)(i / w), (int)(i % w));
        CellIn c;
        c.rho = q[o]; c.jx = q[o + L.plane]; c.jy = q[o + 2 * L.plane];
        c.h = topo[o]; c.hx = topo[o + L.plane]; c.hy = topo[o + 2 * L.plane];
        c.Ls = HAS_LS ? Ls[o] : 0.0;
        CellFields f;
        cell_fields<EOS>(c, P, f);
        F.p[o] = f.p;
        for (int k = 0; k < 3; ++k) F.tau[o + k * L.plane] = f.tau[k];
        for (int k = 0; k < 6; ++k) { F.lower[o + k * L.plane] = f.lower[k]; F.upper[o + k * L.plane] = f.upper[k]; }
    }
}

template <int EOS>
__global__ __launch_bounds__(256) void k_pressure(const double* q, double* p, Layout L, Phys P) {
    const long long w = L.Ny + 2, n = (long long)(L.Nx + 2) * w;
    for (long long i = blockIdx.x * (long long)blockDim.x + threadIdx.x; i < n; i += (long long)gridDim.x * blockDim.x) {
        const long long o = L.at((int)(i / w), (int)(i % w));
        p[o] = eos_pressure<EOS>(q[o], P);
    }
}

template <int EOS, bool HAS_LS>
__global__ __launch_bounds__(256) void k_fields_thinning(const double* q, const double* topo, const double* Ls, FieldPtrs F,
                                                         Layout L, Phys P, double dx, double dy, int halo_lo, int halo_hi,
                                                         const double* beyond) {
    const long long w = L.Ny + 2, n = (long long)(L.Nx + 2) * w;
    for (long long i = blockIdx.x * (long long)blockDim.x + threadIdx.x; i < n; i += (long long)gridDim.x * blockDim.x) {
        const int ix = (int)(i / w), iy = (int)(i % w);
        const long long o = L.at(ix, iy);
        CellIn c;
        c.rho = q[o]; c.jx = q[o + L.plane]; c.jy = q[o + 2 * L.plane];
        c.h = topo[o]; c.hx = topo[o + L.plane]; c.hy = topo[o + 2 * L.plane];
        c.Ls = HAS_LS ? Ls[o] : 0.0;
        const double pc = F.p[o];
        const int ixm = ix > 0 ? ix - 1 : ix, ixp = ix < L.Nx + 1 ? ix + 1 : ix;
        const int iym = iy > 0 ? iy - 1 : iy, iyp = iy < L.Ny + 1 ? iy + 1 : iy;
        double dpx = (F.p[L.at(ixp, iy)] - F.p[L.at(ixm, iy)]) / ((ixp - ixm) * dx);
        if (beyond && ix == 0 && halo_lo == 1)
            dpx = (F.p[L.at(1, iy)] - eos_pressure<EOS>(beyond[L.off + iy], P)) / (2 * dx);
        if (beyond && ix == L.Nx + 1 && halo_hi == 1)
            dpx = (eos_pressure<EOS>(beyond[L.pitch + L.off + iy], P) - F.p[L.at(L.Nx, iy)]) / (2 * dx);
        const double dpy = (F.p[L.at(ix, iyp)] - F.p[L.at(ix, iym)]) / ((iyp - iym) * dy);
        const double mu0 = (P.piezo == PIEZO_NONE) ? P.eta : piezo_eta(P.eta, (EOS == EOS_BAYADA) ? c.rho : pc, P);
        const double eta = thinning_eta(mu0, dpx, dpy, c.h, P);
        CellFields f;
        cell_fields<EOS>(c, P, f, eta);
        for (int k = 0; k < 3; ++k) F.tau[o + k * L.plane] = f.tau[k];
        for (int k = 0; k < 6; ++k) { F.lower[o + k * L.plane] = f.lower[k]; F.upper[o + k * L.plane] = f.upper[k]; }
    }
}

__global__ __launch_bounds__(256) void k_fluxdiff(const double* q, const double* p, const double* tau, int d, double* fx,
                                                  double* fy, Layout L) {
    const long long w = L.Ny + 2, n = (long long)(L.Nx + 2) * w;
    for (long long i = blockIdx.x * (long long)blockDim.x + threadIdx.x; i < n; i += (long long)gridDim.x * blockDim.x) {
        const int ix = (int)(i / w), iy = (int)(i % w);
        const int ixn = (ix - d + (L.Nx + 2)) % (L.Nx + 2);
        const int iyn = (iy - d + (L.Ny + 2)) % (L.Ny + 2);
        const long long o = L.at(ix, iy), ox = L.at(ixn, iy), oy = L.at(ix, iyn);
        const double Fx0 = q[o + L.plane], Fx1 = p[o] + tau[o], Fx2 = tau[o + 2 * L.plane];
        const double Fy0 = q[o + 2 * L.plane], Fy1 = Fx2, Fy2 = p[o] + tau[o + L.plane];
        const double Gx0 = q[ox + L.plane], Gx1 = p[ox] + tau[ox], Gx2 = tau[ox + 2 * L.plane];
        const double Gy0 = q[oy + 2 * L.plane], Gy1 = tau[oy + 2 * L.plane], Gy2 = p[oy] + tau[oy + L.plane];
        const double s = -(double)d;
        fx[o] = s * (Gx0 - Fx0); fx[o + L.plane] = s * (Gx1 - Fx1); fx[o + 2 * L.plane] = s * (Gx2 - Fx2);
        fy[o] = s * (Gy0 - Fy0); fy[o + L.plane] = s * (Gy1 - Fy1); fy[o + 2 * L.plane] = s * (Gy2 - Fy2);
    }
}

__global__ __launch_bounds__(256) void k_source(const double* q, const double* h, const double* tau, const double* lower,
                                                const double* upper, double* out, Layout L) {
    const long long w = L.Ny + 2, n = (long long)(L.Nx + 2) * w, S = L.plane;
    for (long long i = blockIdx.x * (long long)blockDim.x + threadIdx.x; i < n; i += (long long)gridDim.x * blockDim.x) {
        const long long o = L.at((int)(i / w), (int)(i % w));
        const double h0 = h[o], hx = h[o + S], hy = h[o + 2 * S];
        out[o] = (-q[o + S] * hx - q[o + 2 * S] * hy) / h0;
        out[o + S] = ((tau[o] - upper[o]) * hx + (tau[o + 2 * S] - upper[o + 5 * S]) * hy + upper[o + 4 * S] - lower[o + 4 * S]) / h0;
        out[o + 2 * S] = ((tau[o + 2 * S] - upper[o + 5 * S]) * hx + (tau[o + S] - upper[o + S]) * hy + upper[o + 3 * S] - lower[o + 3 * S]) / h0;
    }
}

__global__ __launch_bounds__(256) void k_axpy(double* q, const double* fx, const double* fy, const double* src,
                                              const double* dtp, double dx, double dy, Layout L) {
    const double dt = *dtp;
    const long long w = L.Ny + 2, n = (long long)(L.Nx + 2) * w;
    for (long long i = blockIdx.x * (long long)blockDim.x + threadIdx.x; i < n; i += (long long)gridDim.x * blockDim.x) {
        const long long o = L.at((int)(i / w), (int)(i % w));
        for (int c = 0; c < 3; ++c) {
            const long long oc = o + c * L.plane;
            q[oc] = q[oc] - dt * (fx[oc] / dx + fy[oc] / dy - src[oc]);
        }
    }
}

__global__ __launch_bounds__(256) void k_average(double* q, const double* q0, Layout L) {
    const long long w = L.Ny + 2, n = (long long)(L.Nx + 2) * w;
    for (long long i = blockIdx.x * (long long)blockDim.x + threadIdx.x; i < n; i += (long long)gridDim.x * blockDim.x) {
        const long long o = L.at((int)(i / w), (int)(i % w));
        for (int c = 0; c < 3; ++c) q[o + c * L.plane] = (q[o + c * L.plane] + q0[o + c * L.plane]) / 2.0;
    }
}

__global__ void k_copy3(const double* src, double* dst, long long n) {
    for (long long i = blockIdx.x * (long long)blockDim.x + threadIdx.x; i < n; i += (long long)gridDim.x * blockDim.x)
        dst[i] = src[i];
}

__global__ void k_commit_unfused(StepState* st, const ScalarPartial* pre_bc, const ScalarPartial* post_bc) {
    const int flags = ((int)pre_bc->flags & 3) | ((int)post_bc->flags & 4);
    commit_step(st, post_bc->ekin, post_bc->v2, post_bc->c2, flags, nullptr, 0, 0);
}

struct ViscousArgs {
    const double* q; const double* h; const double* dqx; const double* dqy;
    const double* eta; const double* Ls;
    double U, V, zeta;
    int slip_both;
    double* out[3];
    long long n;
};
__global__ __launch_bounds__(256) void k_viscous(const ViscousArgs a) {
    for (long long i = blockIdx.x * (long long)blockDim.x + threadIdx.x; i < a.n; i += (long long)gridDim.x * blockDim.x) {
        double q[3], h[3], dx[3] = {0.0, 0.0, 0.0}, dy[3] = {0.0, 0.0, 0.0};
        for (int c = 0; c < 3; ++c) {
            q[c] = a.q[c * a.n + i]; h[c] = a.h[c * a.n + i];
            if (a.dqx) dx[c] = a.dqx[c * a.n + i];
            if (a.dqy) dy[c] = a.dqy[c * a.n + i];
        }
        const double Ls = a.Ls[i], lo = a.slip_both ? Ls : 0.0;
        for (int w = 0; w < 3; ++w) {
            if (!a.out[w]) continue;
            double t[6];
            viscous_general(w, q, h, dx, dy, a.U, a.V, a.eta[i], a.zeta, lo, Ls, t);
            if (w < 2) {
                for (int c = 0; c < 6; ++c) a.out[w][c * a.n + i] = t[c];
            } else {
                a.out[2][i] = t[0]; a.out[2][a.n + i] = t[1]; a.out[2][2 * a.n + i] = t[5];
            }
        }
    }
}

template <int EOS>
__global__ __launch_bounds__(256) void k_eos(const double* rho, long long n, Phys P, double* p, double* c) {
    for (long long i = blockIdx.x * (long long)blockDim.x + threadIdx.x; i < n; i += (long long)gridDim.x * blockDim.x) {
        if (p) p[i] = eos_pressure<EOS>(rho[i], P);
        if (c) c[i] = sqrt(eos_c2<EOS>(rho[i], P));
    }
}

__global__ __launch_bounds__(256) void k_viscosity(int kind, const double* a0, const double* a1, const double* a2, long long n,
                                                   double mu0, double u1, double u2, Phys P, double* out) {
    for (long long i = blockIdx.x * (long long)blockDim.x + threadIdx.x; i < n; i += (long long)gridDim.x * blockDim.x) {
        if (kind == 0) out[i] = piezo_eta(mu0, a0[i], P);
        else if (kind == 1) out[i] = thinning_factor(a0[i], mu0, P);
        else out[i] = shear_rate_avg(a0[i], a1[i], a2[i], u1, u2, mu0);
    }
}

}
```

gapflow_amd/csrc/device_types.hpp:

```cpp
#pragma once

#include <stdint.h>
#include "closures.hpp"

namespace gpf {

struct Layout {
    int Nx, Ny;
    int pitch, off;
    long long plane;
    __host__ __device__ __forceinline__ long long at(int ix, int iy) const {
        return (long long)ix * pitch + off + iy;
    }
};

enum { BC_P = 0, BC_D = 1, BC_N = 2 };

struct Edges {
    int rule[4][3];
    double value[4];
    int halo[2];
};

struct StepState {
    double dt;
    double simtime;
    double ekin, ekin_old;
    double residual;
    double vmax2, c2max;
    double rbuf[5];
    int rcount, rhead;
    long long step;
    long long max_it;
    double tol, CFL, hmin;
    int adaptive;
    int mc_order;
    int parity;
    int invalid;
    int converged;
    double dt_last;
};

struct LogEntry {
    long long step;
    double simtime, dt, ekin, ekin_old, residual, v_max, v_sound, mass;
    int invalid, converged;
};

struct Partial {
    double ekin;
    double vmax2;
    double c2max;
    double flags;
};

__host__ __device__ __forceinline__ double nanmax(double m, double x) {
    return (x > m || x != x) ? x : m;
}

}
```

gapflow_amd/csrc/step2_kernel.hip:

```cpp
#include <hip/hip_runtime.h>
#include "device_types.hpp"

namespace gpf {

constexpr int STRIP2 = 126;
#ifndef GPF_K2_AHEAD
#define GPF_K2_AHEAD 2
#endif
#ifndef GPF_K2_AHEAD_LINE
#define GPF_K2_AHEAD_LINE 4
#endif
#ifndef GPF_K2_MINWAVES
#define GPF_K2_MINWAVES 2
#endif
#ifndef GPF_K2_MINWAVES_LINE
#define GPF_K2_MINWAVES_LINE GPF_K2_MINWAVES
#endif
template <int EOS, bool HAS_LS, bool PIEZO>
struct Step2Weight {
    static constexpr bool heavy = EOS == EOS_PL || EOS == EOS_MT || EOS == EOS_BWR || EOS == EOS_BAYADA || (HAS_LS && PIEZO);
};

struct Strip2Geom {
    int w0;
    int nstrips;
    int s_ghost, lane_ghost, slot_ghost;
    int lane_wrap;
    int wrap_ma;
    int wrap_src_lane, wrap_src_slot;
};

struct Step2Args {
    const double* qa; const double* qb;
    const double* topo; const double* topo_line; const double* Ls;
    const double* g1x; const double* g1y;
    const double* seam[2];
    double* out;
    double* msg;
    P2PArgs p2p;
    StepState* st;
    Partial* partials;
    Partial* block_partials;
    unsigned int* arrive;
    LogEntry* log; long long log_base, log_cap;
    Layout L; Edges E; Strip2Geom G;
    int nchunks;
    int fused;
    int honor_stop;
};

__device__ __forceinline__ double lane_from_below(double v) {
#ifdef GPF_SHUFFLE_BPERMUTE
    return __shfl_up(v, 1);
#else
    const long long b = __double_as_longlong(v);
    int lo = (int)b, hi = (int)(b >> 32);
    lo = __builtin_amdgcn_update_dpp(lo, lo, 0x138, 0xf, 0xf, false);
    hi = __builtin_amdgcn_update_dpp(hi, hi, 0x138, 0xf, 0xf, false);
    return __longlong_as_double(((long long)hi << 32) | (unsigned int)lo);
#endif
}
__device__ __forceinline__ double lane_from_above(double v) {
#ifdef GPF_SHUFFLE_BPERMUTE
    return __shfl_down(v, 1);
#else
    const long long b = __double_as_longlong(v);
    int lo = (int)b, hi = (int)(b >> 32);
    lo = __builtin_amdgcn_update_dpp(lo, lo, 0x130, 0xf, 0xf, false);
    hi = __builtin_amdgcn_update_dpp(hi, hi, 0x130, 0xf, 0xf, false);
    return __longlong_as_double(((long long)hi << 32) | (unsigned int)lo);
#endif
}

typedef double dpair __attribute__((ext_vector_type(2)));
#ifndef GPF_K2_NT
#define GPF_K2_NT 2
#endif
__device__ __forceinline__ void asm_load16(dpair& dst, const double* lane_ptr) {
#if GPF_K2_NT & 1
    asm volatile("global_load_dwordx4 %0, %1, off nt" : "=v"(dst) : "v"(lane_ptr) : "memory");
#else
    asm volatile("global_load_dwordx4 %0, %1, off" : "=v"(dst) : "v"(lane_ptr) : "memory");
#endif
}
template <int N>
__device__ __forceinline__ void asm_wait3(dpair& a, dpair& b, dpair& c) {
    asm volatile("s_waitcnt vmcnt(%3)" : "+v"(a), "+v"(b), "+v"(c) : "n"(N) : "memory");
}
template <int N>
__device__ __forceinline__ void asm_wait1(dpair& a) {
    asm volatile("s_waitcnt vmcnt(%1)" : "+v"(a) : "n"(N) : "memory");
}

__device__ __forceinline__ double uniform_load(const double* p) {
    typedef const __attribute__((address_space(4))) double* cptr;
    return *(cptr)(unsigned long long)p;
}

template <int TOPO, bool HAS_LS>
struct RawRow {
    dpair q[3];
    dpair t[TOPO == 0 ? 3 : 1];
    dpair ls[HAS_LS ? 1 : 1];
    double th, thx, thy;
};

struct Row2 { double rho[2], jx[2], jy[2], h[2], hx[2], hy[2], Ls[2]; };

template <int EOS>
struct Red {
    double ekin, v2, c2;
    int flags;
    __device__ __forceinline__ void init() { ekin = 0.0; v2 = 0.0; c2 = (EOS == EOS_DH) ? __builtin_inf() : 0.0; flags = 0; }
    __device__ __forceinline__ void cell(double r, double jx, double jy, double w, const Phys& P) {
        const double v = (jx * jx + jy * jy) * rcp(r);
        ekin += w * (v * 0.5);
        v2 = fmax(v2, v);
        if (v != v) flags |= 1;
        if (r < 0.0) flags |= 2;
        if (EOS == EOS_DH) {
            c2 = fmin(c2, fabs(P.e[7] - r));
        } else {
            const double c = eos_c2<EOS>(r, P);
            if (!(c >= 0.0)) flags |= 4;
            c2 = fmax(c2, c);
        }
    }
};

template <int EOS, bool HAS_LS, bool PIEZO, int D, int TOPO>
__device__ __forceinline__ void step_strip2(const Step2Args& a, const Phys& P, const double* __restrict__ qin,
                                            double* __restrict__ qout, int strip, int chunk, int lane,
                                            double (*stash)[128], Acc& result) {
    const Layout L = a.L;
    const Strip2Geom G = a.G;
    const bool fused = (a.fused & 1) != 0;
    const int policy = __builtin_amdgcn_readfirstlane(a.fused);

    const bool y_periodic = a.E.rule[2][0] == BC_P;
    const bool ghost_strip = strip == G.s_ghost;
    const bool wrap_strip = fused && y_periodic && ghost_strip;
    const bool wrap_lane = wrap_strip && (lane == G.lane_wrap || lane == G.lane_wrap + 1);
    const int ma = wrap_lane ? G.wrap_ma + 2 * (lane - G.lane_wrap) : G.w0 + strip * STRIP2 + 2 * lane;
    const int iy_lo_raw = D > 0 ? ma : L.Ny - ma;
    const bool lane_ok = iy_lo_raw >= -1 && iy_lo_raw <= L.Ny + 1;
    const int iy_lo = lane_ok ? iy_lo_raw : -1;
    const int iy0 = D > 0 ? iy_lo : iy_lo + 1, iy1 = D > 0 ? iy_lo + 1 : iy_lo;
    const bool out0 = lane_ok && !wrap_lane && lane >= 1 && ma >= 1 && ma <= L.Ny;
    const bool out1 = lane_ok && !wrap_lane && lane <= 62 && ma + 1 >= 1 && ma + 1 <= L.Ny;
    const bool is_ghost_lane = ghost_strip && lane == G.lane_ghost;
    const int gsrc_lane = y_periodic ? G.wrap_src_lane : (G.slot_ghost ? G.lane_ghost : G.lane_ghost - 1);
    const int gsrc_slot = y_periodic ? G.wrap_src_slot : (G.slot_ghost ? 0 : 1);

    const int n_first = 1 + (int)(((long long)chunk * L.Nx) / a.nchunks);
    const int n_last = (int)(((long long)(chunk + 1) * L.Nx) / a.nchunks);
    const int e_dw_x = D > 0 ? 1 : 0, e_dw_y = D > 0 ? 3 : 2;
    const bool dw_row_is_ghost = (n_last == L.Nx) && a.E.halo[e_dw_x] != 1;
    const bool x_periodic = a.E.rule[0][0] == BC_P;

    const double dt = a.st->dt;
    const double cx = (double)D * P.inv_dx, cy = (double)D * P.inv_dy;

    const double* __restrict__ q0p = qin;
    const double* __restrict__ q1p = qin + L.plane;
    const double* __restrict__ q2p = qin + 2 * L.plane;
    const double* __restrict__ hp = a.topo;
    const double* __restrict__ hxp = a.topo + L.plane;
    const double* __restrict__ hyp = a.topo + 2 * L.plane;
    double* __restrict__ qo0 = qout;
    double* __restrict__ qo1 = qout + L.plane;
    double* __restrict__ qo2 = qout + 2 * L.plane;

    double lh[2] = {0.0, 0.0}, lhx[2] = {0.0, 0.0}, lhy[2] = {0.0, 0.0};
    if (TOPO == 2) {
        const int c0 = min(max(iy0, 0), L.Ny + 1), c1 = min(max(iy1, 0), L.Ny + 1);
        lh[0] = a.topo_line[c0]; lhx[0] = a.topo_line[(L.Ny + 2) + c0]; lhy[0] = a.topo_line[2 * (L.Ny + 2) + c0];
        lh[1] = a.topo_line[c1]; lhx[1] = a.topo_line[(L.Ny + 2) + c1]; lhy[1] = a.topo_line[2 * (L.Ny + 2) + c1];
    }
    const unsigned int lane_bytes = (unsigned int)(L.off + iy_lo) * 8u;
    auto pair = [&](const double* __restrict__ rowp, double& s0, double& s1) {
        const double2 v = *reinterpret_cast<const double2*>(reinterpret_cast<const char*>(rowp) + lane_bytes);
        s0 = D > 0 ? v.x : v.y; s1 = D > 0 ? v.y : v.x;
    };
    auto load = [&](int n, Row2& r) {
        const int ix = D > 0 ? n : L.Nx + 1 - n;
        const long long rb = (long long)ix * L.pitch;
        pair(q0p + rb, r.rho[0], r.rho[1]); pair(q1p + rb, r.jx[0], r.jx[1]); pair(q2p + rb, r.jy[0], r.jy[1]);
        if (TOPO == 0) {
            pair(hp + rb, r.h[0], r.h[1]); pair(hxp + rb, r.hx[0], r.hx[1]); pair(hyp + rb, r.hy[0], r.hy[1]);
        } else if (TOPO == 1 || TOPO == 3) {
            const double th = a.topo_line[ix], thx = a.topo_line[(L.Nx + 2) + ix], thy = TOPO == 1 ? a.topo_line[2 * (L.Nx + 2) + ix] : 0.0;
            r.h[0] = r.h[1] = th; r.hx[0] = r.hx[1] = thx; r.hy[0] = r.hy[1] = thy;
        } else {
            r.h[0] = lh[0]; r.h[1] = lh[1]; r.hx[0] = lhx[0]; r.hx[1] = lhx[1]; r.hy[0] = lhy[0]; r.hy[1] = lhy[1];
        }
        if (HAS_LS) pair(a.Ls + rb, r.Ls[0], r.Ls[1]);
        else r.Ls[0] = r.Ls[1] = 0.0;
    };
    constexpr int NL = 3 + (TOPO == 0 ? 3 : 0) + (HAS_LS ? 1 : 0);
    typedef RawRow<TOPO, HAS_LS> Raw;
    const double* const lane_q = reinterpret_cast<const double*>(reinterpret_cast<const char*>(qin) + lane_bytes);
    const double* const lane_t = reinterpret_cast<const double*>(reinterpret_cast<const char*>(a.topo) + lane_bytes);
    const double* const lane_ls = HAS_LS ? reinterpret_cast<const double*>(reinterpret_cast<const char*>(a.Ls) + lane_bytes) : nullptr;
    auto issue = [&](int n, Raw& r) {
        const bool dummy = n > n_last + 1;
        const int ix = D > 0 ? min(n, n_last + 1) : L.Nx + 1 - min(n, n_last + 1);
        const long long rb = (long long)ix * L.pitch;
        const long long p1 = dummy ? 0 : L.plane, p2 = dummy ? 0 : 2 * L.plane;
        const double* const a0 = lane_q + rb; const double* const a1 = lane_q + p1 + rb; const double* const a2 = lane_q + p2 + rb;
#define GPF_LD(d, a) "global_load_dwordx4 %" #d ", %" #a ", off\n\t"
#define GPF_LDNT(d, a) "global_load_dwordx4 %" #d ", %" #a ", off nt\n\t"
#define GPF_ROW_HEAD "s_cmp_lg_u32 %[nt], 0\n\ts_cbranch_scc1 .Lgpf_ldnt_%=\n\t"
#define GPF_ROW_MID "s_branch .Lgpf_lddone_%=\n.Lgpf_ldnt_%=:\n\t"
#define GPF_ROW_TAIL "\n.Lgpf_lddone_%=:"
        if constexpr (TOPO == 0 && HAS_LS) {
            const double* t0 = dummy ? lane_q : lane_t;
            const double* const a3 = t0 + rb; const double* const a4 = t0 + p1 + rb; const double* const a5 = t0 + p2 + rb;
            const double* const a6 = (dummy ? lane_q : lane_ls) + rb;
            asm volatile(GPF_ROW_HEAD GPF_LD(0, 7) GPF_LD(1, 8) GPF_LD(2, 9) GPF_LD(3, 10) GPF_LD(4, 11) GPF_LD(5, 12) GPF_LD(6, 13) GPF_ROW_MID
                         GPF_LDNT(0, 7) GPF_LDNT(1, 8) GPF_LDNT(2, 9) GPF_LDNT(3, 10) GPF_LDNT(4, 11) GPF_LDNT(5, 12) GPF_LDNT(6, 13) GPF_ROW_TAIL
                         : "=&v"(r.q[0]), "=&v"(r.q[1]), "=&v"(r.q[2]), "=&v"(r.t[0]), "=&v"(r.t[1]), "=&v"(r.t[2]), "=&v"(r.ls[0])
                         : "v"(a0), "v"(a1), "v"(a2), "v"(a3), "v"(a4), "v"(a5), "v"(a6), [nt] "s"(policy & 4) : "memory", "scc");
        } else if constexpr (TOPO == 0) {
            const double* t0 = dummy ? lane_q : lane_t;
            const double* const a3 = t0 + rb; const double* const a4 = t0 + p1 + rb; const double* const a5 = t0 + p2 + rb;
            asm volatile(GPF_ROW_HEAD GPF_LD(0, 6) GPF_LD(1, 7) GPF_LD(2, 8) GPF_LD(3, 9) GPF_LD(4, 10) GPF_LD(5, 11) GPF_ROW_MID
                         GPF_LDNT(0, 6) GPF_LDNT(1, 7) GPF_LDNT(2, 8) GPF_LDNT(3, 9) GPF_LDNT(4, 10) GPF_LDNT(5, 11) GPF_ROW_TAIL
                         : "=&v"(r.q[0]), "=&v"(r.q[1]), "=&v"(r.q[2]), "=&v"(r.t[0]), "=&v"(r.t[1]), "=&v"(r.t[2])
                         : "v"(a0), "v"(a1), "v"(a2), "v"(a3), "v"(a4), "v"(a5), [nt] "s"(policy & 4) : "memory", "scc");
        } else if constexpr (HAS_LS) {
            const double* const a3 = (dummy ? lane_q : lane_ls) + rb;
            asm volatile(GPF_ROW_HEAD GPF_LD(0, 4) GPF_LD(1, 5) GPF_LD(2, 6) GPF_LD(3, 7) GPF_ROW_MID
                         GPF_LDNT(0, 4) GPF_LDNT(1, 5) GPF_LDNT(2, 6) GPF_LDNT(3, 7) GPF_ROW_TAIL
                         : "=&v"(r.q[0]), "=&v"(r.q[1]), "=&v"(r.q[2]), "=&v"(r.ls[0])
                         : "v"(a0), "v"(a1), "v"(a2), "v"(a3), [nt] "s"(policy & 4) : "memory", "scc");
        } else {
            asm volatile(GPF_ROW_HEAD GPF_LD(0, 3) GPF_LD(1, 4) GPF_LD(2, 5) GPF_ROW_MID GPF_LDNT(0, 3) GPF_LDNT(1, 4) GPF_LDNT(2, 5) GPF_ROW_TAIL
                         : "=&v"(r.q[0]), "=&v"(r.q[1]), "=&v"(r.q[2])
                         : "v"(a0), "v"(a1), "v"(a2), [nt] "s"(policy & 4) : "memory", "scc");
        }
#undef GPF_LD
#undef GPF_LDNT
#undef GPF_ROW_HEAD
#undef GPF_ROW_MID
#undef GPF_ROW_TAIL
        if (TOPO == 1 || TOPO == 3) {
            r.th = uniform_load(a.topo_line + ix); r.thx = uniform_load(a.topo_line + (L.Nx + 2) + ix);
            r.thy = TOPO == 1 ? uniform_load(a.topo_line + 2 * (L.Nx + 2) + ix) : 0.0;
        }
    };
    constexpr bool HEAVY = Step2Weight<EOS, HAS_LS, PIEZO>::heavy;
    constexpr int AHEAD_ROWS = PIEZO ? 1 : (TOPO == 3 ? (HEAVY ? 2 : GPF_K2_AHEAD_LINE) : GPF_K2_AHEAD);
#ifndef GPF_K2_COUNT_STORES
#define GPF_K2_COUNT_STORES 1
#endif
    const bool stores_every_row = GPF_K2_COUNT_STORES && __builtin_amdgcn_ballot_w64(out0 || out1) != 0ull;
    auto arrive = [&](Raw& r, const int n) {
        constexpr int LOOSE = AHEAD_ROWS * NL, EXACT = AHEAD_ROWS * (NL + 3);
        static_assert(EXACT <= 63, "vmcnt is a 6-bit counter");
        const int exact = __builtin_amdgcn_readfirstlane((stores_every_row && n > n_first + AHEAD_ROWS) ? 1 : 0);
#define GPF_WAIT_ROW "s_cmp_lg_u32 %[ex], 0\n\ts_cbranch_scc1 .Lgpf_exact_%=\n\ts_waitcnt vmcnt(%[loose])\n.Lgpf_exact_%=:\n\ts_waitcnt vmcnt(%[exact])"
        if constexpr (TOPO == 0 && HAS_LS)
            asm volatile(GPF_WAIT_ROW : "+v"(r.q[0]), "+v"(r.q[1]), "+v"(r.q[2]), "+v"(r.t[0]), "+v"(r.t[1]), "+v"(r.t[2]), "+v"(r.ls[0])
                         : [ex] "s"(exact), [loose] "n"(LOOSE), [exact] "n"(EXACT) : "memory", "scc");
        else if constexpr (TOPO == 0)
            asm volatile(GPF_WAIT_ROW : "+v"(r.q[0]), "+v"(r.q[1]), "+v"(r.q[2]), "+v"(r.t[0]), "+v"(r.t[1]), "+v"(r.t[2])
                         : [ex] "s"(exact), [loose] "n"(LOOSE), [exact] "n"(EXACT) : "memory", "scc");
        else if constexpr (HAS_LS)
            asm volatile(GPF_WAIT_ROW : "+v"(r.q[0]), "+v"(r.q[1]), "+v"(r.q[2]), "+v"(r.ls[0])
                         : [ex] "s"(exact), [loose] "n"(LOOSE), [exact] "n"(EXACT) : "memory", "scc");
        else
            asm volatile(GPF_WAIT_ROW : "+v"(r.q[0]), "+v"(r.q[1]), "+v"(r.q[2])
                         : [ex] "s"(exact), [loose] "n"(LOOSE), [exact] "n"(EXACT) : "memory", "scc");
#undef GPF_WAIT_ROW
    };
    auto unpack = [&](const Raw& r, Row2& o) {
        o.rho[0] = D > 0 ? r.q[0].x : r.q[0].y; o.rho[1] = D > 0 ? r.q[0].y : r.q[0].x;
        o.jx[0] = D > 0 ? r.q[1].x : r.q[1].y; o.jx[1] = D > 0 ? r.q[1].y : r.q[1].x;
        o.jy[0] = D > 0 ? r.q[2].x : r.q[2].y; o.jy[1] = D > 0 ? r.q[2].y : r.q[2].x;
        if (TOPO == 0) {
            o.h[0] = D > 0 ? r.t[0].x : r.t[0].y; o.h[1] = D > 0 ? r.t[0].y : r.t[0].x;
            o.hx[0] = D > 0 ? r.t[1].x : r.t[1].y; o.hx[1] = D > 0 ? r.t[1].y : r.t[1].x;
            o.hy[0] = D > 0 ? r.t[2].x : r.t[2].y; o.hy[1] = D > 0 ? r.t[2].y : r.t[2].x;
        } else if (TOPO == 1 || TOPO == 3) {
            o.h[0] = o.h[1] = r.th; o.hx[0] = o.hx[1] = r.thx; o.hy[0] = o.hy[1] = r.thy;
        } else {
            o.h[0] = lh[0]; o.h[1] = lh[1]; o.hx[0] = lhx[0]; o.hx[1] = lhx[1]; o.hy[0] = lhy[0]; o.hy[1] = lhy[1];
        }
        if (HAS_LS) { o.Ls[0] = D > 0 ? r.ls[0].x : r.ls[0].y; o.Ls[1] = D > 0 ? r.ls[0].y : r.ls[0].x; }
        else o.Ls[0] = o.Ls[1] = 0.0;
    };
    constexpr bool LS0 = !HAS_LS && !PIEZO;
    auto closure = [&](const Row2& r, int k, const double* q, const TopoRcp& t, const GapCoef& gc, const RowCoef& rc, CellFlux& f) {
        if (TOPO == 3) {
            cell_closure_xonly<EOS>(q ? q[0] : r.rho[k], q ? q[1] : r.jx[k], q ? q[2] : r.jy[k], rc, P, f);
        } else if (LS0) {
            cell_closure_ls0<EOS>(q ? q[0] : r.rho[k], q ? q[1] : r.jx[k], q ? q[2] : r.jy[k], gc, P, f);
        } else {
            CellIn c;
            c.rho = q ? q[0] : r.rho[k]; c.jx = q ? q[1] : r.jx[k]; c.jy = q ? q[2] : r.jy[k];
            c.h = r.h[k]; c.hx = r.hx[k]; c.hy = r.hy[k]; c.Ls = r.Ls[k];
            cell_closure<EOS, true, HAS_LS, PIEZO>(c, t, P, f);
        }
    };
    auto cell_of = [&](const Row2& r, int k) {
        CellIn c;
        c.rho = r.rho[k]; c.jx = r.jx[k]; c.jy = r.jy[k]; c.h = r.h[k]; c.hx = r.hx[k]; c.hy = r.hy[k]; c.Ls = r.Ls[k];
        return c;
    };

    Red<EOS> red;
    red.init();
    const int seam_row_lo = a.E.halo[0] == 2 ? 1 : -1, seam_row_hi = a.E.halo[1] == 2 ? L.Nx : -1;

    if (fused && dw_row_is_ghost && x_periodic) {
        Row2 r0, r1;
        if (a.E.halo[e_dw_x] == 2) {
            load(L.Nx, r0);
            load(L.Nx + 1, r1);
            auto seam_topo = [&](const double* __restrict__ t, Row2& r) {
                if (TOPO == 1 || TOPO == 3) {
                    r.h[0] = r.h[1] = t[L.off + 1]; r.hx[0] = r.hx[1] = t[L.pitch + L.off + 1];
                    r.hy[0] = r.hy[1] = TOPO == 1 ? t[2 * L.pitch + L.off + 1] : 0.0;
                } else {
                    pair(t, r.h[0], r.h[1]); pair(t + L.pitch, r.hx[0], r.hx[1]); pair(t + 2 * L.pitch, r.hy[0], r.hy[1]);
                }
                if (HAS_LS) pair(t + 3 * L.pitch, r.Ls[0], r.Ls[1]);
            };
            seam_topo(a.seam[e_dw_x] + 4 * L.pitch, r0);
            seam_topo(a.seam[e_dw_x], r1);
        } else {
            load(0, r0);
            load(1, r1);
        }
        double fy[2][3], q1[2][3];
        CellFlux f0[2], f1[2];
        const RowCoef rc0 = TOPO == 3 ? row_coefficients(r0.h[0], r0.hx[0], P) : RowCoef();
        const RowCoef rc1 = TOPO == 3 ? row_coefficients(r1.h[0], r1.hx[0], P) : RowCoef();
        for (int k = 0; k < 2; ++k) {
            closure(r0, k, nullptr, topo_rcp<HAS_LS>(cell_of(r0, k)), gap_coefficients(r0.h[k], r0.hx[k], r0.hy[k]), rc0, f0[k]);
            closure(r1, k, nullptr, topo_rcp<HAS_LS>(cell_of(r1, k)), gap_coefficients(r1.h[k], r1.hx[k], r1.hy[k]), rc1, f1[k]);
            fy[k][0] = r1.jy[k]; fy[k][1] = f1[k].fx2; fy[k][2] = f1[k].fy2;
        }
        const double u0 = lane_from_below(fy[1][0]), u1 = lane_from_below(fy[1][1]), u2 = lane_from_below(fy[1][2]);
        const double up[2][3] = {{u0, u1, u2}, {fy[0][0], fy[0][1], fy[0][2]}};
        for (int k = 0; k < 2; ++k) {
            q1[k][0] = predictor_value(r1.rho[k], dt, cx, r1.jx[k] - r0.jx[k], cy, fy[k][0] - up[k][0], f1[k].s0);
            q1[k][1] = predictor_value(r1.jx[k], dt, cx, f1[k].fx1 - f0[k].fx1, cy, fy[k][1] - up[k][1], f1[k].s1);
            q1[k][2] = predictor_value(r1.jy[k], dt, cx, f1[k].fx2 - f0[k].fx2, cy, fy[k][2] - up[k][2], f1[k].s2);
            for (int c = 0; c < 3; ++c) stash[c][2 * lane + k] = q1[k][c];
        }
    }

    if (!fused && dw_row_is_ghost) {
        const int c0 = min(max(iy0, 0), L.Ny + 1), c1 = min(max(iy1, 0), L.Ny + 1);
        for (int c = 0; c < 3; ++c) {
            stash[c][2 * lane] = a.g1x[c * L.pitch + L.off + c0];
            stash[c][2 * lane + 1] = a.g1x[c * L.pitch + L.off + c1];
        }
    }

    constexpr int AHEAD = AHEAD_ROWS;
    static_assert(AHEAD >= 1 && AHEAD <= 6, "1 to 6 rows ahead");
    constexpr int NB = AHEAD + 1;
    Raw rowbuf[NB];
    issue(n_first - 1, rowbuf[0]);
    if (AHEAD >= 2) issue(n_first, rowbuf[1 % NB]);
    if (AHEAD >= 3) issue(n_first + 1, rowbuf[2 % NB]);
    if (AHEAD >= 4) issue(n_first + 2, rowbuf[3 % NB]);
    if (AHEAD >= 5) issue(n_first + 3, rowbuf[4 % NB]);
    if (AHEAD >= 6) issue(n_first + 4, rowbuf[5 % NB]);

    double fx1p[2][3] = {{0, 0, 0}, {0, 0, 0}};
    double part[2][3] = {{0, 0, 0}, {0, 0, 0}};

    auto march = [&](const int n, Raw& raw, Raw& spare) {
        issue(n + AHEAD, spare);
        arrive(raw, n);
        Row2 cur;
        unpack(raw, cur);
        const bool first = (n == n_first - 1);
        const bool last = (n == n_last + 1);
        const int ix = D > 0 ? n : L.Nx + 1 - n;

        TopoRcp tr[2] = {TopoRcp(), TopoRcp()};
        GapCoef gc[2] = {GapCoef(), GapCoef()};
        RowCoef rc = RowCoef();
        if (TOPO == 3) {
            rc = row_coefficients(cur.h[0], cur.hx[0], P);
        } else if (LS0) {
            gc[0] = gap_coefficients(cur.h[0], cur.hx[0], cur.hy[0]);
            gc[1] = gap_coefficients(cur.h[1], cur.hx[1], cur.hy[1]);
        } else {
            tr[0] = topo_rcp<HAS_LS>(cell_of(cur, 0));
            tr[1] = topo_rcp<HAS_LS>(cell_of(cur, 1));
        }

        double q1[2][3];
        if (last && dw_row_is_ghost) {
            for (int k = 0; k < 2; ++k)
                for (int c = 0; c < 3; ++c) q1[k][c] = stash[c][2 * lane + k];
        } else {
            CellFlux f[2];
            double fy[2][3];
            for (int k = 0; k < 2; ++k) {
                closure(cur, k, nullptr, tr[k], gc[k], rc, f[k]);
                fy[k][0] = cur.jy[k]; fy[k][1] = f[k].fx2; fy[k][2] = f[k].fy2;
            }
            const double u0 = lane_from_below(fy[1][0]), u1 = lane_from_below(fy[1][1]), u2 = lane_from_below(fy[1][2]);
            const double up[2][3] = {{u0, u1, u2}, {fy[0][0], fy[0][1], fy[0][2]}};
            for (int k = 0; k < 2; ++k) {
                q1[k][0] = predictor_value(cur.rho[k], dt, cx, cur.jx[k] - fx1p[k][0], cy, fy[k][0] - up[k][0], f[k].s0);
                q1[k][1] = predictor_value(cur.jx[k], dt, cx, f[k].fx1 - fx1p[k][1], cy, fy[k][1] - up[k][1], f[k].s1);
                q1[k][2] = predictor_value(cur.jy[k], dt, cx, f[k].fx2 - fx1p[k][2], cy, fy[k][2] - up[k][2], f[k].s2);
                fx1p[k][0] = cur.jx[k]; fx1p[k][1] = f[k].fx1; fx1p[k][2] = f[k].fx2;
            }
            if (ghost_strip) {
                double gv[3];
                if (!fused) {
                    for (int c = 0; c < 3; ++c) gv[c] = uniform_load(a.g1y + c * (L.Nx + 2) + ix);
                } else {
                    for (int c = 0; c < 3; ++c)
                        gv[c] = ghost_rule(a.E, e_dw_y, c, __shfl(gsrc_slot ? q1[1][c] : q1[0][c], gsrc_lane));
                }
                if (is_ghost_lane) {
                    for (int c = 0; c < 3; ++c) {
                        if (G.slot_ghost) q1[1][c] = gv[c];
                        else q1[0][c] = gv[c];
                    }
                }
            }
            if (fused && n == n_last && dw_row_is_ghost && !x_periodic) {
                for (int k = 0; k < 2; ++k)
                    for (int c = 0; c < 3; ++c) stash[c][2 * lane + k] = ghost_rule(a.E, e_dw_x, c, q1[k][c]);
            }
        }

        if (!first) {
            CellFlux g[2];
            double gy[2][3];
            for (int k = 0; k < 2; ++k) {
                closure(cur, k, q1[k], tr[k], gc[k], rc, g[k]);
                gy[k][0] = q1[k][2]; gy[k][1] = g[k].fx2; gy[k][2] = g[k].fy2;
            }
            const double d0 = lane_from_above(gy[0][0]), d1 = lane_from_above(gy[0][1]), d2 = lane_from_above(gy[0][2]);
            const double dn[2][3] = {{gy[1][0], gy[1][1], gy[1][2]}, {d0, d1, d2}};

            if (n > n_first) {
                double o[2][3];
                for (int k = 0; k < 2; ++k) {
                    o[k][0] = 0.5 * (part[k][0] - dt * cx * q1[k][1]);
                    o[k][1] = 0.5 * (part[k][1] - dt * cx * g[k].fx1);
                    o[k][2] = 0.5 * (part[k][2] - dt * cx * g[k].fx2);
                }
                const int ixo = D > 0 ? n - 1 : L.Nx + 2 - n;
                const long long rbo = (long long)ixo * L.pitch;
#if GPF_K2_NT & 2
                const bool store_nt = (policy & 2) && (ixo & 7) >= ((policy >> 3) & 7);
#endif
                auto st16 = [&](double* __restrict__ rowp, double va, double vb) {
                    dpair v;
                    v.x = D > 0 ? va : vb; v.y = D > 0 ? vb : va;
                    dpair* p = reinterpret_cast<dpair*>(reinterpret_cast<char*>(rowp) + lane_bytes);
#if GPF_K2_NT & 2
                    asm volatile("s_cmp_lg_u32 %[nt], 0\n\ts_cbranch_scc1 .Lgpf_stnt_%=\n\t"
                                 "global_store_dwordx4 %0, %1, off\n\ts_branch .Lgpf_stdone_%=\n"
                                 ".Lgpf_stnt_%=:\n\tglobal_store_dwordx4 %0, %1, off nt\n"
                                 ".Lgpf_stdone_%=:\n\ts_nop 0"
                                 :: "v"(p), "v"(v), [nt] "s"(__builtin_amdgcn_readfirstlane(store_nt ? 1 : 0)) : "memory", "scc");
#else
                    *p = v;
#endif
                };
                auto st8 = [&](double* __restrict__ rowp, unsigned int bytes, double v) {
                    *reinterpret_cast<double*>(reinterpret_cast<char*>(rowp) + bytes) = v;
                };
                if (out0 && out1) {
                    st16(qo0 + rbo, o[0][0], o[1][0]); st16(qo1 + rbo, o[0][1], o[1][1]); st16(qo2 + rbo, o[0][2], o[1][2]);
                } else if (out0) {
                    const unsigned int b = (unsigned int)(L.off + iy0) * 8u;
                    st8(qo0 + rbo, b, o[0][0]); st8(qo1 + rbo, b, o[0][1]); st8(qo2 + rbo, b, o[0][2]);
                } else if (out1) {
                    const unsigned int b = (unsigned int)(L.off + iy1) * 8u;
                    st8(qo0 + rbo, b, o[1][0]); st8(qo1 + rbo, b, o[1][1]); st8(qo2 + rbo, b, o[1][2]);
                }
                const double w = 1.0 + (ixo == seam_row_lo ? 1.0 : 0.0) + (ixo == seam_row_hi ? 1.0 : 0.0);
                if (out0) red.cell(o[0][0], o[0][1], o[0][2], w, P);
                if (out1) red.cell(o[1][0], o[1][1], o[1][2], w, P);
            }
            for (int k = 0; k < 2; ++k) {
                part[k][0] = (cur.rho[k] + q1[k][0]) - dt * (-cx * q1[k][1] + cy * (dn[k][0] - gy[k][0]) - g[k].s0);
                part[k][1] = (cur.jx[k] + q1[k][1]) - dt * (-cx * g[k].fx1 + cy * (dn[k][1] - gy[k][1]) - g[k].s1);
                part[k][2] = (cur.jy[k] + q1[k][2]) - dt * (-cx * g[k].fx2 + cy * (dn[k][2] - gy[k][2]) - g[k].s2);
            }
        }
    };
    for (int n = n_first - 1;;) {
        march(n, rowbuf[0], rowbuf[AHEAD]); if (++n > n_last + 1) break;
        march(n, rowbuf[1], rowbuf[0]); if (++n > n_last + 1) break;
        if (AHEAD >= 2) { march(n, rowbuf[2 % NB], rowbuf[1]); if (++n > n_last + 1) break; }
        if (AHEAD >= 3) { march(n, rowbuf[3 % NB], rowbuf[2 % NB]); if (++n > n_last + 1) break; }
        if (AHEAD >= 4) { march(n, rowbuf[4 % NB], rowbuf[3 % NB]); if (++n > n_last + 1) break; }
        if (AHEAD >= 5) { march(n, rowbuf[5 % NB], rowbuf[4 % NB]); if (++n > n_last + 1) break; }
        if (AHEAD >= 6) { march(n, rowbuf[6 % NB], rowbuf[5 % NB]); if (++n > n_last + 1) break; }
    }
    for (int b = 0; b <= AHEAD; ++b) {
        asm_wait3<0>(rowbuf[b].q[0], rowbuf[b].q[1], rowbuf[b].q[2]);
        if (TOPO == 0) asm_wait3<0>(rowbuf[b].t[0], rowbuf[b].t[1], rowbuf[b].t[2]);
        if (HAS_LS) asm_wait1<0>(rowbuf[b].ls[0]);
    }

#ifndef GPF_K2_NO_POSTPASS
    if (fused) {
        asm volatile("s_waitcnt vmcnt(0)" ::: "memory");
        const int src_row[2] = {x_periodic ? L.Nx : 1, x_periodic ? 1 : L.Nx};
        const int src_col[2] = {y_periodic ? L.Ny : 1, y_periodic ? 1 : L.Ny};
        const int ix_lo = D > 0 ? n_first : L.Nx + 1 - n_last, ix_hi = D > 0 ? n_last : L.Nx + 1 - n_first;
        auto get = [&](int ix, int iy, double v[3]) {
            const long long o = (long long)ix * L.pitch + L.off + iy;
            v[0] = qo0[o]; v[1] = qo1[o]; v[2] = qo2[o];
        };
        auto put = [&](int ix, int iy, const double v[3], double w) {
            const long long o = (long long)ix * L.pitch + L.off + iy;
            qo0[o] = v[0]; qo1[o] = v[1]; qo2[o] = v[2];
            red.cell(v[0], v[1], v[2], w, P);
        };
        double* send_to[2] = {nullptr, nullptr};
        if (a.p2p.on) {
            const int slot = (int)((*a.p2p.seq + 1) & 1);
            if (a.E.halo[0] && a.p2p.rank_lo >= 0) send_to[0] = p2p_rows(a.p2p.box[a.p2p.rank_lo], slot, 1, L.pitch);
            if (a.E.halo[1] && a.p2p.rank_hi >= 0) send_to[1] = p2p_rows(a.p2p.box[a.p2p.rank_hi], slot, 0, L.pitch);
        } else if (a.msg) {
            if (a.E.halo[0]) send_to[0] = a.msg;
            if (a.E.halo[1]) send_to[1] = a.msg + 3 * L.pitch;
        }
        auto send = [&](int e, int iy, const double v[3]) {
            double* d = send_to[e] + L.off + iy;
            for (int c = 0; c < 3; ++c) {
                if (a.p2p.on)
                    __hip_atomic_store(reinterpret_cast<unsigned long long*>(d + c * L.pitch), (unsigned long long)__double_as_longlong(v[c]),
                                       __ATOMIC_RELAXED, __HIP_MEMORY_SCOPE_SYSTEM);
                else d[c * L.pitch] = v[c];
            }
        };
        const int m_out_lo = max(G.w0 + strip * STRIP2 + 1, 1), m_out_hi = min(G.w0 + strip * STRIP2 + STRIP2, L.Ny);
        for (int ey = 0; ey < 2; ++ey) {
            const int msrc = D > 0 ? src_col[ey] : L.Ny + 1 - src_col[ey];
            if (msrc < m_out_lo || msrc > m_out_hi) continue;
            for (int ix = ix_lo + lane; ix <= ix_hi; ix += 64) {
                double v[3], g[3];
                get(ix, src_col[ey], v);
                for (int c = 0; c < 3; ++c) g[c] = ghost_rule(a.E, 2 + ey, c, v[c]);
                put(ix, ey ? L.Ny + 1 : 0, g, 1.0 + (ix == seam_row_lo ? 1.0 : 0.0) + (ix == seam_row_hi ? 1.0 : 0.0));
                if (ix == 1 && send_to[0]) send(0, ey ? L.Ny + 1 : 0, g);
                if (ix == L.Nx && send_to[1]) send(1, ey ? L.Ny + 1 : 0, g);
            }
        }
        for (int e = 0; e < 2; ++e) {
            if (a.E.halo[e]) continue;
            if (src_row[e] < ix_lo || src_row[e] > ix_hi) continue;
            const int ixg = e ? L.Nx + 1 : 0;
            for (int k = 0; k < 2; ++k) {
                if (!(k ? out1 : out0)) continue;
                const int iy = k ? iy1 : iy0;
                double v[3], g[3], gc[3];
                get(src_row[e], iy, v);
                for (int c = 0; c < 3; ++c) g[c] = ghost_rule(a.E, e, c, v[c]);
                put(ixg, iy, g, 1.0);
                for (int ey = 0; ey < 2; ++ey) {
                    if (iy != src_col[ey]) continue;
                    for (int c = 0; c < 3; ++c) gc[c] = ghost_rule(a.E, 2 + ey, c, g[c]);
                    put(ixg, ey ? L.Ny + 1 : 0, gc, 1.0);
                }
            }
        }
        for (int e = 0; e < 2; ++e) {
            const int ixb = e ? L.Nx : 1;
            if (!send_to[e] || ixb < ix_lo || ixb > ix_hi) continue;
            for (int k = 0; k < 2; ++k) {
                if (!(k ? out1 : out0)) continue;
                double v[3];
                get(ixb, k ? iy1 : iy0, v);
                send(e, k ? iy1 : iy0, v);
            }
        }
        if (a.p2p.on) asm volatile("s_waitcnt vmcnt(0)" ::: "memory");
    }
#endif

    for (int s = 32; s >= 1; s >>= 1) {
        red.ekin += __shfl_down(red.ekin, s);
        red.v2 = fmax(red.v2, __shfl_down(red.v2, s));
        const double oc = __shfl_down(red.c2, s);
        red.c2 = (EOS == EOS_DH) ? fmin(red.c2, oc) : fmax(red.c2, oc);
        red.flags |= __shfl_down(red.flags, s);
    }
    if (EOS == EOS_DH) {
        const double it = rcp(red.c2);
        red.c2 = (red.c2 == __builtin_inf()) ? 0.0 : P.e[6] * (it * it);
    }
#ifdef GPF_K2_NO_POSTPASS
    red.flags = 0;
#endif
    result.ekin = red.ekin; result.v2 = red.v2; result.c2 = red.c2; result.mass = 0.0; result.flags = red.flags;
}

template <int EOS, bool HAS_LS, bool PIEZO, int D, int TOPO>
__global__ __launch_bounds__(256, (Step2Weight<EOS, HAS_LS, PIEZO>::heavy ? 1 : ((TOPO == 1 || TOPO == 3) ? GPF_K2_MINWAVES_LINE : GPF_K2_MINWAVES)))
void k_step2(const Step2Args a, const Phys P) {
    __shared__ double stash[4][3][128];
    __shared__ Acc red_sm[4];
    __shared__ int s_last;
    if (halted(a.st, a.honor_stop)) return;
    if (predictor_direction(a.st) != D) __builtin_trap();
    const int par = a.st->parity;
    const double* qin = par ? a.qb : a.qa;
    double* qout = const_cast<double*>(par ? a.qa : a.qb);

    const int nb = gridDim.x;
    const int lb = (int)(blockIdx.x & 7) * (nb >> 3) + (int)(blockIdx.x >> 3);
    const int wv = __builtin_amdgcn_readfirstlane(threadIdx.x >> 6), lane = threadIdx.x & 63;
    const int w = lb * 4 + wv;
    const int strip = w % a.G.nstrips, chunk = w / a.G.nstrips;
    const bool active = chunk < a.nchunks;

    Acc own;
    own.zero();
    if (active) step_strip2<EOS, HAS_LS, PIEZO, D, TOPO>(a, P, qin, qout, strip, chunk, lane, stash[wv], own);

    if (!(a.fused & 1)) {
        if (active && lane == 0) {
            Partial p;
            p.ekin = own.ekin; p.vmax2 = own.v2; p.c2max = own.c2; p.flags = (double)own.flags;
            a.partials[w] = p;
        }
        return;
    }
#ifdef GPF_K2_NO_FINISH
    if (blockIdx.x == 0 && threadIdx.x == 0) commit_step(a.st, own.ekin + 1.0, own.v2, own.c2, own.flags, a.log, a.log_base, a.log_cap);
    return;
#endif
    if (lane == 0) red_sm[wv] = own;
    __syncthreads();
    if (threadIdx.x == 0) {
        Acc tot = red_sm[0];
        for (int i = 1; i < 4; ++i) { tot.ekin += red_sm[i].ekin; tot.v2 = fmax(tot.v2, red_sm[i].v2); tot.c2 = fmax(tot.c2, red_sm[i].c2); tot.flags |= red_sm[i].flags; }
        publish_partial(a.block_partials + blockIdx.x, tot);
        const unsigned int t = __hip_atomic_fetch_add(a.arrive, 1u, GPF_ORDER_ARRIVE, __HIP_MEMORY_SCOPE_AGENT);
        s_last = (t == (unsigned int)nb - 1) ? 1 : 0;
        if (s_last) __hip_atomic_store(a.arrive, 0u, __ATOMIC_RELAXED, __HIP_MEMORY_SCOPE_AGENT);
    }
    __syncthreads();
    if (!s_last) return;
    finish_tail(a.st, a.log, a.log_base, a.log_cap, a.out, a.block_partials, a.p2p, red_sm);
}

}
```

Before: 120,400 Mcell-updates/s.

## Defer step commit to next launch head instead of last-block atomic tail

Replaces the end-of-kernel atomic arrival counter and last-block finish tail with a head-commit scheme. Each block writes its partial reduction to a double-buffered array, and the next launch folds the previous partials at its start to commit the step state and derive dt, overlapping this with the first row prefetches. A trailing commit kernel closes each batch. This removes the serialized last-block tail and atomic contention per step, but every block redundantly re-reduces all previous partials at launch head and adds host-side parity tracking.

```diff
diff --git a/gapflow_amd/csrc/api.hip b/gapflow_amd/csrc/api.hip
--- a/gapflow_amd/csrc/api.hip
+++ b/gapflow_amd/csrc/api.hip
@@ -131,6 +131,12 @@
     int nt_policy2 = 0;
     int keep_rows2 = 0;
     StepState* st_trial = nullptr;
+    bool head_commit = true;
+    StepState* st_slots = nullptr;
+    int batch_launch = -1;
+    int batch_parity0 = 0;
+    bool parity_known = false;
+    int host_parity = 0;
     double* plan_master = nullptr;
     char plan2_note[400] = "";
 };
@@ -138,6 +144,7 @@
 static int enter(gpf_handle* h, bool reads_only) {
     HIP_TRY(hipSetDevice(h->cfg.device));
     if (!reads_only) h->gp_state_mean_valid = false;
+    h->parity_known = false;
     return GPF_OK;
 }
 
@@ -267,7 +274,14 @@
     h->nghost_blocks = std::max(1, std::min(64, (2 * (L.Ny + 2) + 2 * L.Nx + 255) / 256));
     HIP_TRY_C(hipMalloc(&h->arrive, 4 * sizeof(unsigned int)));
     HIP_TRY_C(hipMemset(h->arrive, 0, 4 * sizeof(unsigned int)));
-    HIP_TRY_C(hipMalloc(&h->block_partials, 1024 * sizeof(Partial)));
+    HIP_TRY_C(hipMalloc(&h->block_partials, (size_t)4 * 1024 * sizeof(Partial)));
+    h->nblock_partials_cap = 1024;
+    HIP_TRY_C(hipMalloc(&h->st_slots, 4 * sizeof(StepState)));
+    HIP_TRY_C(hipMemset(h->st_slots, 0, 4 * sizeof(StepState)));
+    if (const char* e = std::getenv("GPF_HEAD_COMMIT")) h->head_commit = std::atoi(e) != 0;
+#ifdef GPF_K2_NO_FINISH
+    h->head_commit = false;
+#endif
     h->nspart = 1024;
     HIP_TRY_C(hipMalloc(&h->spart, (size_t)(h->nspart + 8) * sizeof(ScalarPartial)));
     HIP_TRY_C(hipMemset(h->spart, 0, (size_t)(h->nspart + 8) * sizeof(ScalarPartial)));
@@ -284,7 +298,7 @@
     hipStreamSynchronize(h->stream);
     for (void* p : {(void*)h->q[0], (void*)h->q[1], (void*)h->topo, (void*)h->plan_master}) field_free(p);
     void* ptrs[] = {h->topo_line, h->Ls, h->g1, h->seam, h->halo, h->beyond, h->st, h->partials, h->arrive, h->block_partials, h->spart,
-                    h->log, h->stage, h->fields, h->work, h->st_trial, h->gpvar, h->gp_state_mean, h->gpscratch, h->gptile,
+                    h->log, h->stage, h->fields, h->work, h->st_trial, h->st_slots, h->gpvar, h->gp_state_mean, h->gpscratch, h->gptile,
                     h->gp[0].Z, h->gp[0].alpha, h->gp[0].L, h->gp[1].Z, h->gp[1].alpha, h->gp[1].L,
                     h->gp[2].Z, h->gp[2].alpha, h->gp[2].L, h->gp[0].Linv, h->gp[1].Linv, h->gp[2].Linv, h->gp[0].W, h->gp[1].W, h->gp[2].W};
     if (h->blas && roclibs().ok) roclibs().destroy(h->blas);
@@ -572,6 +586,7 @@
 }
 
 static int write_state(gpf_handle* h, const StepState& s) {
+    h->parity_known = false;
     HIP_TRY(hipMemcpyAsync(h->st, &s, sizeof(s), hipMemcpyHostToDevice, h->stream));
     HIP_TRY(hipStreamSynchronize(h->stream));
     return GPF_OK;
@@ -708,7 +723,7 @@
     return GPF_OK;
 }
 
-static void fill_step2_args(gpf_handle* h, Step2Args& a2, int D, int honor_stop, long long log_base, double* slab_out, bool p2p) {
+static void fill_step2_args(gpf_handle* h, Step2Args& a2, int D, int honor_stop, long long log_base, double* slab_out, bool p2p, int head_launch) {
     const Layout& L = h->L;
     const bool fused = step2_fused(h);
     const Strip2Geom& G2 = h->geom2[D > 0 ? 0 : 1];
@@ -721,6 +736,39 @@
     const bool slab = slab_out != nullptr;
     for (int e = 0; e < 2; ++e) a2.seam[e] = (h->E.halo[e] == 2 && h->has_seam[e]) ? h->seam + (size_t)e * 8 * L.pitch : nullptr;
     a2.out = slab_out; a2.msg = (slab && !p2p) ? h->halo : nullptr; a2.p2p = p2p_args(h, p2p);
+    a2.st_out = nullptr; a2.rec_in = nullptr;
+    if (head_launch >= 0) {
+        const int i = head_launch;
+        const size_t cap = (size_t)h->nblock_partials_cap;
+        a2.fused |= K2_HEAD_COMMIT | (((h->batch_parity0 ^ i) & 1) << K2_PARITY_SHIFT);
+        a2.st = i == 0 ? h->st : h->st_slots + (i & 1);
+        a2.st_out = h->st_slots + ((i + 1) & 1);
+        a2.rec_in = h->block_partials + ((i + 1) & 1) * cap;
+        a2.block_partials = h->block_partials + (i & 1) * cap;
+    }
+}
+
+static bool head_commit_on(const gpf_handle* h) { return h->head_commit && step2_fused(h) && !h->E.halo[0] && !h->E.halo[1]; }
+
+static int open_batch(gpf_handle* h) {
+    h->batch_launch = -1;
+    if (!head_commit_on(h)) return GPF_OK;
+    if (!h->parity_known) {
+        GPF_TRY(current_parity(h, &h->host_parity));
+        h->parity_known = true;
+    }
+    h->batch_parity0 = h->host_parity;
+    h->batch_launch = 0;
+    return GPF_OK;
+}
+static int close_batch(gpf_handle* h, long long log_base) {
+    const int n = h->batch_launch;
+    h->batch_launch = -1;
+    if (n <= 0) return GPF_OK;
+    hipLaunchKernelGGL(k_commit_pending, dim3(1), dim3(256), 0, h->stream, (const StepState*)(h->st_slots + (n & 1)),
+                       (const Partial*)(h->block_partials + (size_t)((n - 1) & 1) * h->nblock_partials_cap), h->st, h->log, log_base, h->log_cap);
+    HIP_TRY(hipGetLastError());
+    return GPF_OK;
 }
 
 static int enqueue_step(gpf_handle* h, int honor_stop, long long log_base, double* slab_out,
@@ -735,9 +783,10 @@
     const int np_step = G2.nstrips * h->nchunks2;
     GhostArgs g;
     GPF_TRY(ghost_args(h, honor_stop, g));
+    const bool slab = slab_out != nullptr;
+    const int head_launch = (h->batch_launch >= 0 && !slab && !p2p && head_commit_on(h)) ? h->batch_launch++ : -1;
     Step2Args a2;
-    fill_step2_args(h, a2, D, honor_stop, log_base, slab_out, p2p);
-    const bool slab = slab_out != nullptr;
+    fill_step2_args(h, a2, D, honor_stop, log_base, slab_out, p2p, head_launch);
     FinishArgs f;
     f.partials = h->partials; f.st = h->st;
     f.log = h->log; f.log_base = log_base; f.log_cap = h->log_cap; f.out = slab_out; f.honor_stop = honor_stop;
@@ -827,6 +876,7 @@
     if (h->cfg.thinning != GPF_THINNING_NONE)
         return fail(GPF_ERR_STATE, "gpf_step: shear thinning needs grad p (a wider stencil than the fused step has); use the stage-wise calls");
     if (n < 0) return fail(GPF_ERR_INVALID, "gpf_step: n < 0");
+    bool parity_known = h->parity_known;
     GPF_TRY(enter(h));
     int64_t done = 0, logged = 0;
     const bool small = small_grid_eligible(h);
@@ -834,9 +884,18 @@
         const int64_t batch = std::min<int64_t>(n - done, h->log_cap);
         const long long base = h->host_step;
         if (small) GPF_TRY(enqueue_small_steps(h, (int)batch, honor_stop, base));
-        else for (int64_t i = 0; i < batch; ++i) GPF_TRY(enqueue_step(h, honor_stop, base, nullptr));
+        else {
+            h->parity_known = parity_known;
+            GPF_TRY(open_batch(h));
+            int rc = GPF_OK;
+            for (int64_t i = 0; i < batch && rc == GPF_OK; ++i) rc = enqueue_step(h, honor_stop, base, nullptr);
+            GPF_TRY(close_batch(h, base));
+            GPF_TRY(rc);
+        }
         StepState s;
         GPF_TRY(read_state(h, s));
+        if (s.invalid == INVALID_HOST_DESYNC) return fail(GPF_ERR_STATE, "gpf_step: a step was enqueued for another direction or buffer than the device state says");
+        h->host_parity = s.parity; parity_known = !small;
         const long long ran = s.step - base;
         const long long entries = ran + ((s.invalid && ran < batch) ? 1 : 0);
         if (log && entries > 0) {
@@ -852,6 +911,7 @@
         if (ran < batch) break;
     }
     if (n_executed) *n_executed = h->host_step;
+    h->parity_known = parity_known;
     return GPF_OK;
 }
 
@@ -862,9 +922,11 @@
     GPF_TRY(enter(h));
     std::vector<hipEvent_t> ev(2 * n + 2);
     for (auto& e : ev) HIP_TRY(hipEventCreate(&e));
+    GPF_TRY(open_batch(h));
     HIP_TRY(hipEventRecord(ev[2 * n], h->stream));
     int rc = GPF_OK;
     for (int64_t i = 0; i < n && rc == GPF_OK; ++i) rc = enqueue_step(h, 0, h->host_step, nullptr, ev[2 * i], ev[2 * i + 1]);
+    GPF_TRY(close_batch(h, h->host_step));
     HIP_TRY(hipEventRecord(ev[2 * n + 1], h->stream));
     HIP_TRY(hipStreamSynchronize(h->stream));
     double sum = 0.0;
@@ -880,6 +942,8 @@
     GPF_TRY(read_state(h, s));
     h->prev_state_valid = s.step > h->host_step && !s.invalid;
     h->host_step = s.step; h->next_step = s.step;
+    h->host_parity = s.parity; h->parity_known = true;
+    if (s.invalid == INVALID_HOST_DESYNC) return fail(GPF_ERR_STATE, "gpf_step_timed: a step was enqueued for another direction or buffer than the device state says");
     return rc;
 }
 
diff --git a/gapflow_amd/csrc/api_plan.inc b/gapflow_amd/csrc/api_plan.inc
--- a/gapflow_amd/csrc/api_plan.inc
+++ b/gapflow_amd/csrc/api_plan.inc
@@ -21,13 +21,15 @@
         const int cap = std::max(1024, h->nblocks2);
         if (h->block_partials) HIP_TRY(hipFree(h->block_partials));
         h->block_partials = nullptr;
-        HIP_TRY(hipMalloc(&h->block_partials, (size_t)cap * sizeof(Partial)));
+        HIP_TRY(hipMalloc(&h->block_partials, (size_t)4 * cap * sizeof(Partial)));
         h->nblock_partials_cap = cap;
     }
     return GPF_OK;
 }
 
-static void fill_step2_args(gpf_handle* h, Step2Args& a2, int D, int honor_stop, long long log_base, double* slab_out, bool p2p);
+static void fill_step2_args(gpf_handle* h, Step2Args& a2, int D, int honor_stop, long long log_base, double* slab_out, bool p2p, int head_launch);
+static bool head_commit_on(const gpf_handle* h);
+static int read_state(gpf_handle* h, StepState& s);
 
 static int plan_trial(gpf_handle* h, int D, float* us, int reps = 6, bool both = false) {
     static const int parity_value[2] = {0, 1};
@@ -37,16 +39,37 @@
     int par = 0;
     if (both) GPF_TRY(current_parity(h, &par));
     Step2Args a2;
-    fill_step2_args(h, a2, D, 0, 0, nullptr, false);
+    fill_step2_args(h, a2, D, 0, 0, nullptr, false, -1);
     a2.st = h->st_trial; a2.log = nullptr;
+    const bool head = head_commit_on(h);
+    StepState s_now, s_back[2];
+    if (head) {
+        GPF_TRY(read_state(h, s_now));
+        par = s_now.parity;
+        for (int flip = 0; flip < 2; ++flip) {
+            s_back[flip] = s_now;
+            s_back[flip].step -= 1; s_back[flip].parity = par ^ flip ^ 1; s_back[flip].pending = h->nblocks2;
+        }
+        a2.fused |= K2_HEAD_COMMIT;
+        a2.st = h->st_slots + 2; a2.st_out = h->st_slots + 3;
+    }
     const step2_kernel_t k2 = step2_kernel(h->cfg.eos, h->Ls != nullptr, h->cfg.piezo != 0, D, topo_mode_of(h));
     hipEvent_t e0, e1;
     HIP_TRY(hipEventCreate(&e0)); HIP_TRY(hipEventCreate(&e1));
     float total = 0.f;
     for (int r = -1; r < reps; ++r) {
+        if (head) {
+            const int flip = (both && ((r + 1) & 1)) ? 1 : 0;
+            const size_t cap = (size_t)h->nblock_partials_cap;
+            HIP_TRY(hipMemcpyAsync(h->st_slots + 2, r < 0 ? &s_now : &s_back[flip], sizeof(StepState), hipMemcpyHostToDevice, h->stream));
+            a2.fused = (a2.fused & ~(1 << K2_PARITY_SHIFT)) | ((par ^ flip) << K2_PARITY_SHIFT);
+            a2.rec_in = h->block_partials + 2 * cap;
+            a2.block_partials = h->block_partials + (r < 0 ? 2 : 3) * cap;
+        } else {
         HIP_TRY(hipMemcpyAsync(h->st_trial, h->st, sizeof(StepState), hipMemcpyDeviceToDevice, h->stream));
         if (both && ((r + 1) & 1))
             HIP_TRY(hipMemcpyAsync(&h->st_trial->parity, &parity_value[par ^ 1], sizeof(int), hipMemcpyHostToDevice, h->stream));
+        }
         HIP_TRY(hipEventRecord(e0, h->stream));
         hipLaunchKernelGGL(k2, dim3(h->nblocks2), dim3(256), 0, h->stream, a2, h->P);
         HIP_TRY(hipEventRecord(e1, h->stream));
diff --git a/gapflow_amd/csrc/aux_kernels.hip b/gapflow_amd/csrc/aux_kernels.hip
--- a/gapflow_amd/csrc/aux_kernels.hip
+++ b/gapflow_amd/csrc/aux_kernels.hip
@@ -131,40 +131,47 @@
     return st->hmin / (sqrt(v2) + sqrt(c2));
 }
 
-__device__ inline void commit_step(StepState* st, double ekin, double v2, double c2, int flags, LogEntry* log,
-                                   long long log_base, long long log_cap) {
+__device__ inline int commit_compute(StepState& s, double ekin, double v2, double c2, int flags) {
     if (flags & 4) c2 = __builtin_nan("");
     flags &= 3;
     if (flags) {
-        st->invalid = (flags & 1) ? 1 : 2;
+        s.invalid = (flags & 1) ? 1 : 2;
     } else {
-        const double dt_crit = critical_dt(st, v2, c2);
-        const double cfl = st->dt / dt_crit;
-        const double res = fabs(ekin - st->ekin_old) / st->ekin_old / cfl;
-        st->residual = res;
-        if (st->rcount < 5) { st->rbuf[st->rcount++] = res; }
-        else { st->rbuf[st->rhead] = res; st->rhead = (st->rhead + 1) % 5; }
+        const double dt_crit = critical_dt(&s, v2, c2);
+        const double cfl = s.dt / dt_crit;
+        const double res = fabs(ekin - s.ekin_old) / s.ekin_old / cfl;
+        s.residual = res;
+        if (s.rcount < 5) { s.rbuf[s.rcount++] = res; }
+        else { s.rbuf[s.rhead] = res; s.rhead = (s.rhead + 1) % 5; }
         bool conv = true;
-        for (int i = 0; i < st->rcount; ++i) conv = conv && (st->rbuf[i] < st->tol);
-        st->converged = conv ? 1 : 0;
-        st->ekin_old = ekin;
-        st->ekin = ekin; st->vmax2 = v2; st->c2max = c2;
-        st->step += 1;
-        st->simtime += st->dt;
-        st->dt_last = st->dt;
-        if (st->adaptive) st->dt = st->CFL * dt_crit;
-        st->parity ^= 1;
-    }
+        for (int i = 0; i < s.rcount; ++i) conv = conv && (s.rbuf[i] < s.tol);
+        s.converged = conv ? 1 : 0;
+        s.ekin_old = ekin;
+        s.ekin = ekin; s.vmax2 = v2; s.c2max = c2;
+        s.step += 1;
+        s.simtime += s.dt;
+        s.dt_last = s.dt;
+        if (s.adaptive) s.dt = s.CFL * dt_crit;
+        s.parity ^= 1;
+    }
+    return flags;
+}
+__device__ inline void commit_log(const StepState& s, int flags, LogEntry* log, long long log_base, long long log_cap) {
     if (log) {
-        const long long k = (flags ? st->step : st->step - 1) - log_base;
+        const long long k = (flags ? s.step : s.step - 1) - log_base;
         if (k >= 0 && k < log_cap) {
             LogEntry e;
-            e.step = st->step; e.simtime = st->simtime; e.dt = st->dt; e.ekin = st->ekin; e.ekin_old = st->ekin_old;
-            e.residual = st->residual; e.v_max = sqrt(st->vmax2); e.v_sound = sqrt(st->c2max); e.mass = 0.0;
-            e.invalid = st->invalid; e.converged = st->converged;
+            e.step = s.step; e.simtime = s.simtime; e.dt = s.dt; e.ekin = s.ekin; e.ekin_old = s.ekin_old;
+            e.residual = s.residual; e.v_max = sqrt(s.vmax2); e.v_sound = sqrt(s.c2max); e.mass = 0.0;
+            e.invalid = s.invalid; e.converged = s.converged;
             log[k] = e;
         }
     }
+}
+__device__ inline void commit_step(StepState* st, double ekin, double v2, double c2, int flags, LogEntry* log,
+                                   long long log_base, long long log_cap) {
+    const int rolled_back = commit_compute(*st, ekin, v2, c2, flags);
+    commit_log(*st, rolled_back, log, log_base, log_cap);
 }
 
 constexpr long long P2P_TIMEOUT_TICKS = 3000000000ll;
@@ -258,6 +265,39 @@
 
 __device__ inline void finish_tail(const FinishArgs& a, Acc* sm) {
     finish_tail(a.st, a.log, a.log_base, a.log_cap, a.out, a.block_partials, a.p2p, sm);
+}
+
+constexpr int INVALID_PEER_TIMEOUT = 3;
+constexpr int INVALID_HOST_DESYNC = 4;
+__device__ __forceinline__ void merge_record(Acc& acc, const Partial& p) {
+    acc.ekin += p.ekin; acc.v2 = nanmax(acc.v2, p.vmax2); acc.c2 = nanmax(acc.c2, p.c2max); acc.flags |= (int)p.flags;
+}
+__device__ __forceinline__ Acc fold_records(const Partial* rec, int n, Acc* sm) {
+    Acc acc; acc.zero();
+    if (n > 0) {
+        for (int i = threadIdx.x; i < n; i += blockDim.x) merge_record(acc, rec[i]);
+        acc = block_reduce(acc, sm);
+    }
+    return acc;
+}
+__device__ __forceinline__ void commit_pending(StepState& s, const StepState* in, const Acc& acc, bool writer, LogEntry* log,
+                                               long long log_base, long long log_cap) {
+    s = *in;
+    if (s.pending > 0) {
+        const int rolled_back = commit_compute(s, acc.ekin, acc.v2, acc.c2, acc.flags);
+        if (writer) commit_log(s, rolled_back, log, log_base, log_cap);
+    }
+    s.pending = 0;
+}
+__global__ __launch_bounds__(256) void k_commit_pending(const StepState* in, const Partial* rec, StepState* out, LogEntry* log,
+                                                        long long log_base, long long log_cap) {
+    __shared__ Acc sm[4];
+    __shared__ StepState s;
+    const Acc acc = fold_records(rec, in->pending, sm);
+    if (threadIdx.x == 0) {
+        commit_pending(s, in, acc, true, log, log_base, log_cap);
+        *out = s;
+    }
 }
 
 __device__ inline void finish_step(const FinishArgs& f, Acc own, Acc* sm) {
@@ -414,7 +454,6 @@
     if (i < n) state[i] = (work[i] + state[i]) / 2.0;
 }
 
-constexpr int INVALID_PEER_TIMEOUT = 3;
 struct WaitArgs {
     double* qa; double* qb;
     StepState* st;
diff --git a/gapflow_amd/csrc/device_types.hpp b/gapflow_amd/csrc/device_types.hpp
--- a/gapflow_amd/csrc/device_types.hpp
+++ b/gapflow_amd/csrc/device_types.hpp
@@ -39,6 +39,7 @@
     int invalid;
     int converged;
     double dt_last;
+    int pending;
 };
 
 struct LogEntry {
diff --git a/gapflow_amd/csrc/step2_kernel.hip b/gapflow_amd/csrc/step2_kernel.hip
--- a/gapflow_amd/csrc/step2_kernel.hip
+++ b/gapflow_amd/csrc/step2_kernel.hip
@@ -4,6 +4,7 @@
 namespace gpf {
 
 constexpr int STRIP2 = 126;
+constexpr int K2_HEAD_COMMIT = 64, K2_PARITY_SHIFT = 7;
 #ifndef GPF_K2_AHEAD
 #define GPF_K2_AHEAD 2
 #endif
@@ -39,6 +40,8 @@
     double* msg;
     P2PArgs p2p;
     StepState* st;
+    StepState* st_out;
+    const Partial* rec_in;
     Partial* partials;
     Partial* block_partials;
     unsigned int* arrive;
@@ -86,6 +89,9 @@
 template <int N>
 __device__ __forceinline__ void asm_wait3(dpair& a, dpair& b, dpair& c) {
     asm volatile("s_waitcnt vmcnt(%3)" : "+v"(a), "+v"(b), "+v"(c) : "n"(N) : "memory");
+}
+__device__ __forceinline__ void asm_drain3(const dpair& a, const dpair& b, const dpair& c) {
+    asm volatile("s_waitcnt vmcnt(0)" :: "v"(a), "v"(b), "v"(c) : "memory");
 }
 template <int N>
 __device__ __forceinline__ void asm_wait1(dpair& a) {
@@ -128,10 +134,10 @@
     }
 };
 
-template <int EOS, bool HAS_LS, bool PIEZO, int D, int TOPO>
-__device__ __forceinline__ void step_strip2(const Step2Args& a, const Phys& P, const double* __restrict__ qin,
+template <int EOS, bool HAS_LS, bool PIEZO, int D, int TOPO, class Head>
+__device__ __forceinline__ bool step_strip2(const Step2Args& a, const Phys& P, const double* __restrict__ qin,
                                             double* __restrict__ qout, int strip, int chunk, int lane,
-                                            double (*stash)[128], Acc& result) {
+                                            double (*stash)[128], Acc& result, Head&& head) {
     const Layout L = a.L;
     const Strip2Geom G = a.G;
     const bool fused = (a.fused & 1) != 0;
@@ -158,7 +164,7 @@
     const bool dw_row_is_ghost = (n_last == L.Nx) && a.E.halo[e_dw_x] != 1;
     const bool x_periodic = a.E.rule[0][0] == BC_P;
 
-    const double dt = a.st->dt;
+    double dt = (a.fused & K2_HEAD_COMMIT) ? 0.0 : a.st->dt;
     const double cx = (double)D * P.inv_dx, cy = (double)D * P.inv_dy;
 
     const double* __restrict__ q0p = qin;
@@ -313,8 +319,37 @@
     red.init();
     const int seam_row_lo = a.E.halo[0] == 2 ? 1 : -1, seam_row_hi = a.E.halo[1] == 2 ? L.Nx : -1;
 
-    if (fused && dw_row_is_ghost && x_periodic) {
-        Row2 r0, r1;
+    if (!fused && dw_row_is_ghost) {
+        const int c0 = min(max(iy0, 0), L.Ny + 1), c1 = min(max(iy1, 0), L.Ny + 1);
+        for (int c = 0; c < 3; ++c) {
+            stash[c][2 * lane] = a.g1x[c * L.pitch + L.off + c0];
+            stash[c][2 * lane + 1] = a.g1x[c * L.pitch + L.off + c1];
+        }
+    }
+
+    constexpr int AHEAD = AHEAD_ROWS;
+    static_assert(AHEAD >= 1 && AHEAD <= 6, "1 to 6 rows ahead");
+    constexpr int NB = AHEAD + 1;
+    Raw rowbuf[NB];
+    issue(n_first - 1, rowbuf[0]);
+    if (AHEAD >= 2) issue(n_first, rowbuf[1 % NB]);
+    if (AHEAD >= 3) issue(n_first + 1, rowbuf[2 % NB]);
+    if (AHEAD >= 4) issue(n_first + 2, rowbuf[3 % NB]);
+    if (AHEAD >= 5) issue(n_first + 3, rowbuf[4 % NB]);
+    if (AHEAD >= 6) issue(n_first + 4, rowbuf[5 % NB]);
+
+    if (!head(dt)) {
+        for (int b = 0; b <= AHEAD; ++b) {
+            asm_drain3(rowbuf[b].q[0], rowbuf[b].q[1], rowbuf[b].q[2]);
+            if (TOPO == 0) asm_drain3(rowbuf[b].t[0], rowbuf[b].t[1], rowbuf[b].t[2]);
+            if (HAS_LS) asm_drain3(rowbuf[b].ls[0], rowbuf[b].ls[0], rowbuf[b].ls[0]);
+        }
+        return false;
+    }
+
+    const bool ghost_row_prologue = fused && dw_row_is_ghost && x_periodic;
+    Row2 r0, r1;
+    if (ghost_row_prologue) {
         if (a.E.halo[e_dw_x] == 2) {
             load(L.Nx, r0);
             load(L.Nx + 1, r1);
@@ -333,6 +368,9 @@
             load(0, r0);
             load(1, r1);
         }
+    }
+
+    if (ghost_row_prologue) {
         double fy[2][3], q1[2][3];
         CellFlux f0[2], f1[2];
         const RowCoef rc0 = TOPO == 3 ? row_coefficients(r0.h[0], r0.hx[0], P) : RowCoef();
@@ -352,24 +390,6 @@
         }
     }
 
-    if (!fused && dw_row_is_ghost) {
-        const int c0 = min(max(iy0, 0), L.Ny + 1), c1 = min(max(iy1, 0), L.Ny + 1);
-        for (int c = 0; c < 3; ++c) {
-            stash[c][2 * lane] = a.g1x[c * L.pitch + L.off + c0];
-            stash[c][2 * lane + 1] = a.g1x[c * L.pitch + L.off + c1];
-        }
-    }
-
-    constexpr int AHEAD = AHEAD_ROWS;
-    static_assert(AHEAD >= 1 && AHEAD <= 6, "1 to 6 rows ahead");
-    constexpr int NB = AHEAD + 1;
-    Raw rowbuf[NB];
-    issue(n_first - 1, rowbuf[0]);
-    if (AHEAD >= 2) issue(n_first, rowbuf[1 % NB]);
-    if (AHEAD >= 3) issue(n_first + 1, rowbuf[2 % NB]);
-    if (AHEAD >= 4) issue(n_first + 2, rowbuf[3 % NB]);
-    if (AHEAD >= 5) issue(n_first + 3, rowbuf[4 % NB]);
-    if (AHEAD >= 6) issue(n_first + 4, rowbuf[5 % NB]);
 
     double fx1p[2][3] = {{0, 0, 0}, {0, 0, 0}};
     double part[2][3] = {{0, 0, 0}, {0, 0, 0}};
@@ -603,6 +623,7 @@
     red.flags = 0;
 #endif
     result.ekin = red.ekin; result.v2 = red.v2; result.c2 = red.c2; result.mass = 0.0; result.flags = red.flags;
+    return true;
 }
 
 template <int EOS, bool HAS_LS, bool PIEZO, int D, int TOPO>
@@ -611,9 +632,17 @@
     __shared__ double stash[4][3][128];
     __shared__ Acc red_sm[4];
     __shared__ int s_last;
-    if (halted(a.st, a.honor_stop)) return;
-    if (predictor_direction(a.st) != D) __builtin_trap();
-    const int par = a.st->parity;
+    __shared__ StepState s_st;
+    __shared__ int s_go;
+    const bool head_commit = (a.fused & K2_HEAD_COMMIT) != 0;
+    int par;
+    if (head_commit) {
+        par = (a.fused >> K2_PARITY_SHIFT) & 1;
+    } else {
+        if (halted(a.st, a.honor_stop)) return;
+        if (predictor_direction(a.st) != D) __builtin_trap();
+        par = a.st->parity;
+    }
     const double* qin = par ? a.qb : a.qa;
     double* qout = const_cast<double*>(par ? a.qa : a.qb);
 
@@ -624,9 +653,28 @@
     const int strip = w % a.G.nstrips, chunk = w / a.G.nstrips;
     const bool active = chunk < a.nchunks;
 
+    auto head = [&](double& dt) -> bool {
+        if (!head_commit) return true;
+        const Acc acc = fold_records(a.rec_in, a.st->pending, red_sm);
+        if (threadIdx.x == 0) {
+            commit_pending(s_st, a.st, acc, blockIdx.x == 0, a.log, a.log_base, a.log_cap);
+            if (!halted(&s_st, a.honor_stop) && (predictor_direction(&s_st) != D || s_st.parity != par)) s_st.invalid = INVALID_HOST_DESYNC;
+            const int go = halted(&s_st, a.honor_stop) ? 0 : 1;
+            s_st.pending = go ? (int)gridDim.x : 0;
+            s_go = go;
+            if (blockIdx.x == 0) *a.st_out = s_st;
+        }
+        __syncthreads();
+        dt = s_st.dt;
+        return s_go != 0;
+    };
     Acc own;
     own.zero();
-    if (active) step_strip2<EOS, HAS_LS, PIEZO, D, TOPO>(a, P, qin, qout, strip, chunk, lane, stash[wv], own);
+    bool go;
+    double dt_unused;
+    if (active) go = step_strip2<EOS, HAS_LS, PIEZO, D, TOPO>(a, P, qin, qout, strip, chunk, lane, stash[wv], own, head);
+    else go = head(dt_unused);
+    if (__builtin_amdgcn_readfirstlane(go ? 1 : 0) == 0) return;
 
     if (!(a.fused & 1)) {
         if (active && lane == 0) {
@@ -642,9 +690,16 @@
 #endif
     if (lane == 0) red_sm[wv] = own;
     __syncthreads();
+    if (head_commit && threadIdx.x != 0) return;
     if (threadIdx.x == 0) {
         Acc tot = red_sm[0];
         for (int i = 1; i < 4; ++i) { tot.ekin += red_sm[i].ekin; tot.v2 = fmax(tot.v2, red_sm[i].v2); tot.c2 = fmax(tot.c2, red_sm[i].c2); tot.flags |= red_sm[i].flags; }
+        if (head_commit) {
+            Partial p;
+            p.ekin = tot.ekin; p.vmax2 = tot.v2; p.c2max = tot.c2; p.flags = (double)tot.flags;
+            a.block_partials[blockIdx.x] = p;
+            return;
+        }
         publish_partial(a.block_partials + blockIdx.x, tot);
         const unsigned int t = __hip_atomic_fetch_add(a.arrive, 1u, GPF_ORDER_ARRIVE, __HIP_MEMORY_SCOPE_AGENT);
         s_last = (t == (unsigned int)nb - 1) ? 1 : 0;
```

Measured after the change: 120,600 Mcell-updates/s (median of 3 runs). About the same (+0.2%).
